# powei-lin/aprilgrid-rs

Hardware: AMD Instinct MI355X
Metric: Mpix/s through the saddle chain (blur->threshold->gradient->saddle), frames resident in HBM (higher is better)
Workload: dtype f32; 1 GPU; configs[1]: 256 synthetic 1280x800 L8 AprilGrid frames per GPU (T36H11 6x6 board, seeded renderer, frame indices 0..255 per rank: 256 distinct); frames_per_gpu=256, width=1280, height=800, format=L8, distinct_frames_per_gpu=256, parallelism=1 GPU, steps_per_gather=1, batches_in_flight=1

## Files before the change

### aprilgrid-rs_amd/csrc/chain_kernels.h

```cpp
#pragma once
#include <cstddef>
#include <cstdint>

namespace agx {

enum Kernel : int {
    K_BLUR_HESSIAN = 0,
    K_THRESHOLD = 1,
    K_FLOOD_REFINE = 2,
    K_RARE = 3,
    K_SPARSE = 4,
    K_COUNT = 5
};

struct RefinedRec {
    uint32_t key;
    float x, y, k, theta, phi;
};

struct FrameCounters {
    uint32_t min_key_inv;
    uint32_t pad0[31];
    uint32_t n_seeds;
    uint32_t n_clusters;
    uint32_t n_refined;
    uint32_t max_k_bits;
    uint32_t flags;
    uint32_t n_out;
    uint32_t out_offset;
    uint32_t n_cand;
    uint32_t n_roots;
    uint32_t n_big;
    uint32_t refine_done;
    uint32_t n_clusters2;
    uint32_t stats[20];
};
static_assert(sizeof(FrameCounters) == 256, "FrameCounters is cleared as 64 dwords");
enum : uint32_t {
    FLAG_CAND_OVERFLOW = 1u,
    FLAG_ROOT_OVERFLOW = 2u,
    FLAG_OUT_OVERFLOW = 4u,
    FLAG_CENTROID_INEXACT = 8u,
    FLAG_BIG_CLUSTER = 16u,
    FLAG_RING_BELOW = 32u,
    FLAG_LARGE_RESULT = 64u
};

struct RefineConsts {
    float cone[25];
    float pmat[150];
};

struct ChainArgs {
    const uint8_t *frames;
    long long frame_stride;
    int row_stride;
    int byte_rows;
    int fmt;
    int W, H, n_frames;
    long long plane;
    int threads;
    int n_strips;
    int strip_cols;
    int rows_per_seg;
    int n_segs;
    int k1_group;
    int k1_async_poll;
    float publish_factor;
    float w[7];
    float *blur;
    float *resp_dbg;
    float *dummy;
    float *cand_max;
    uint32_t *slot_plane;
    uint32_t *mask;
    int mask_wpr;
    int mask_yb;
    long long mask_plane;
    int force_generic;
    int sparse_after_verify;
    unsigned long long *wave_times;
    int dbg;
    FrameCounters *ctr;
    FrameCounters *ctr_next;
    uint32_t *total_out;
    uint32_t cap_cand, cap_roots, cap_out;
    uint32_t *seeds;
    uint32_t *clu_key;
    uint32_t *clu_cnt;
    uint32_t *clu_sx, *clu_sy;
    uint32_t *cand;
    uint32_t *parent;
    unsigned long long *sumx, *sumy;
    uint32_t *cnt, *minidx;
    uint32_t *roots;
    RefinedRec *refined;
    float *out;
    uint32_t out_total_cap;
    uint32_t *frame_table;
    float min_angle, max_angle;
};

int tuning_env(const char *name, int dflt);
void tuning_env_reload();

bool plan_k1(ChainArgs &a, int override_rows_per_seg);

int launch_kernel(int which, const ChainArgs &a, const RefineConsts &rc, void *stream, bool deferred_refine = false);

struct RefinePointsArgs {
    const float *img;
    long long frame_stride;
    long long pitch;
    int W, H;
    int padded;
    const float *points;
    uint32_t points_per_frame;
    const uint32_t *counts;
    float *out;
    uint32_t *status;
};
int launch_refine_points(const RefinePointsArgs &p, const RefineConsts &rc, int n_frames, void *stream);

constexpr int REFINE_PATCH_MAX_HALF = 4;
constexpr int REFINE_PATCH_MAX_TAPS = (2 * REFINE_PATCH_MAX_HALF + 1) * (2 * REFINE_PATCH_MAX_HALF + 1);
struct RefinePatchConsts {
    float cone[REFINE_PATCH_MAX_TAPS];
    float pmat[REFINE_PATCH_MAX_TAPS * 6];
};
int launch_refine_patch(const RefinePointsArgs &p, const RefinePatchConsts *consts, int half, int n_frames, void *stream);

int launch_generic_cluster(const ChainArgs &a, void *stream);
int launch_refine_clusters(const ChainArgs &a, const RefinePatchConsts *consts, int half, void *stream);

size_t k5_lds_bytes(const ChainArgs &a);

constexpr size_t WAVE_TIMES_STRIDE = (size_t)1 << 20;

constexpr int MASK_PAD_X = 64;

int init_device_kernels();

int launch_debug_resp(const ChainArgs &a, int frame, float *dst, void *stream);
int launch_publish(const ChainArgs &a, uint32_t h_out_records, uint32_t *h_table_dev, float *h_out_dev, void *stream);
int launch_clear_counters(FrameCounters *ctr, size_t n_records, void *stream);
int launch_front_luma(const void *src, size_t row_stride, size_t frame_stride, int n_frames, int format, void *dst, int out8, int W,
                      int H, void *stream);
int launch_luma8(const void *src, size_t pitch, size_t frame_stride, int n_frames, int format, uint8_t *dst, int W, int H,
                 void *stream);


constexpr int GB_MAX_RADIUS = 16;
constexpr int GB_TX = 64, GB_TY = 64;
constexpr int GB_HPITCH = GB_TX + 1;
struct GaussBlurArgs {
    const uint8_t *src;
    long long src_frame_stride;
    int src_row_stride;
    int W, H;
    float *dst;
    long long dst_frame_stride;
    long long dst_row_stride;
    int radius;
    float w[2 * GB_MAX_RADIUS + 1];
};
size_t gauss_blur_lds_bytes(int radius);
int launch_gauss_blur(const GaussBlurArgs &a, int format, int n_frames, void *stream);

struct HessianArgs {
    const uint8_t *src;
    long long src_frame_stride;
    int src_row_stride;
    int W, H;
    float *dst;
    long long dst_frame_stride, dst_row_stride;
};
int launch_hessian_response(const HessianArgs &a, int format, int n_frames, void *stream);

int launch_response_front(const ChainArgs &a, void *stream);

struct PlaneFrontArgs {
    const float *src;
    long long frame_stride;
    long long row_stride;
};
int launch_plane_front(const ChainArgs &a, const PlaneFrontArgs &p, void *stream);

constexpr uint32_t EMIT_CLUSTERS_MAX = 16384;
struct EmitClustersArgs {
    uint32_t per_frame;
    uint32_t *rows;
    float *points;
    uint32_t *counts;
    uint32_t *status;
};
int launch_emit_clusters(const ChainArgs &a, const EmitClustersArgs &e, void *stream);

struct FilterSaddlesArgs {
    const float *records;
    uint32_t *status;
    const uint32_t *counts;
    uint32_t per_frame;
    float min_angle, max_angle;
    uint32_t filtered;
};
int launch_filter_saddles(const FilterSaddlesArgs &f, int n_frames, void *stream);

}
```

### aprilgrid-rs_amd/csrc/chain_kernels.hip

```cpp
#include <hip/hip_runtime.h>

#include <map>
#include <mutex>
#include <string>

#include "chain_kernels.h"

namespace agx {

__device__ __forceinline__ uint32_t f32_order_key(float f)
{
    uint32_t u = __float_as_uint(f);
    return (u & 0x80000000u) ? ~u : (u | 0x80000000u);
}
__device__ __forceinline__ float f32_from_order_key(uint32_t key)
{
    uint32_t u = (key & 0x80000000u) ? (key & 0x7fffffffu) : ~key;
    return __uint_as_float(u);
}

template <int D>
__device__ __forceinline__ float div_const(float v)
{
    const float r = 1.0f / (float)D;
// ... 642 lines not shown
                            s_def[wv][y - ys][lane_id_here()] = pk;
                        }
                        if (cj_any != 0ull && !defer_row) {
                            float sel[4];
#pragma unroll
                            for (int j = 0; j < 4; ++j)
                                asm("v_cndmask_b32_e64 %0, %1, %2, %3" : "=v"(sel[j]) : "v"(cmax), "v"(dv[j]), "s"(cj[j]));
                            cmax = fmaxf(fmaxf(cmax, sel[0]), sel[1]);
                            cmax = fmaxf(fmaxf(cmax, sel[2]), sel[3]);
                        }
                    }
                    y_pushed = y;
                }
                if (__builtin_expect((y & 31) == 31 || y == ye - 1, 0)) {
                    const int ln = lane_id_here();
                    const int c0h = xs - 4 + 4 * ln;
                    auto store_block = [&](int yb, const uint32_t (&w)[4], float m) {
                        if (c0h >= xs && c0h < xe) {
                            a.cand_max[((size_t)frame * a.mask_yb + yb) * (a.mask_wpr >> 2) + ((MASK_PAD_X + c0h) >> 2)] = m;
                            uint32_t *dst = mask_f + (size_t)yb * a.mask_wpr + MASK_PAD_X + c0h;
                            if (A4) {
                                *reinterpret_cast<uint4 *>(dst) = make_uint4(w[0], w[1], w[2], w[3]);
                            } else {
#pragma unroll
                                for (int j = 0; j < 4; ++j)
                                    if (c0h + j < W) dst[j] = w[j];
                            }
                        }
                    };
                    auto refilter = [&](uint32_t (&w)[4], float &m) {
                        const float thr_now = __builtin_bit_cast(float, thr_run_bits);
                        const int q_lo = ys < 1 ? 1 - ys : 0;
                        const int q_hi = min(K1_DEFER_ROWS, min(ye, H - 1) - ys);
#pragma unroll 1
                        for (int q = q_lo; q < q_hi; ++q) {
                            const uint2 pk = s_def[wv][q][ln];
#pragma unroll
                            for (int j = 0; j < 4; ++j) {
                                const uint32_t half = j < 2 ? pk.x : pk.y;
                                const uint32_t raw = (j & 1) ? (half & 0xffff0000u) : (half << 16);
                                const float hi = __uint_as_float(raw), lo = __uint_as_float(raw | 0xffffu);
                                const bool bit = ((w[j] >> q) & 1u) != 0u;
                                const bool keep = bit && lo < thr_now;
                                if (bit && !keep) w[j] &= ~(1u << q);
                                if (keep) m = fmaxf(m, hi);
                            }
                        }
                    };
                    const int blk = (y >> 5) - (ys >> 5);
                    if (DEFER && blk == 1) {
                        uint32_t o0[4];
#pragma unroll
                        for (int j = 0; j < 4; ++j) o0[j] = s_blk0[wv][j][ln];
                        float cm0 = __uint_as_float(s_blk0[wv][4][ln]);
                        refilter(o0, cm0);
                        store_block((y >> 5) - 1, o0, cm0);
                    }
                    const int fix = 31 - (y_pushed & 31);
#pragma unroll
                    for (int j = 0; j < 4; ++j) mw[j] = __brev(mw[j]) >> fix;
                    if (DEFER && blk == 0 && y != ye - 1) {
#pragma unroll
                        for (int j = 0; j < 4; ++j) s_blk0[wv][j][ln] = mw[j];
                        s_blk0[wv][4][ln] = __float_as_uint(cmax);
                    } else {
                        if (DEFER && blk == 0) refilter(mw, cmax);
                        store_block(y >> 5, mw, cmax);
                    }
                    mw[0] = mw[1] = mw[2] = mw[3] = 0u;
                    cmax = -__builtin_inff();
                }
            }
            up = mid;
            mid = dn;
        }
    }
    const float run_min = wave_min_f32(lane_min());
    if (async_poll) polled = __builtin_amdgcn_readfirstlane(polled_v);
    else if (first_sync) asm volatile("s_waitcnt lgkmcnt(0)" : "+s"(polled) : : "memory");
    const bool known_smaller = polled != 0u && !(run_min < f32_from_order_key(~polled));
    if (lane == 0 && !known_smaller) atomicMax(&ctr.min_key_inv, ~f32_order_key(run_min));
}

__device__ __forceinline__ float det_at(const float *c, int W)
{
    const float v11 = c[-W - 1], v12 = c[-W], v13 = c[-W + 1];
    const float v21 = c[-1], v22 = c[0], v23 = c[1];
    const float v31 = c[W - 1], v32 = c[W], v33 = c[W + 1];
    const float t22 = v22 * 2.0f;
    const float lxx = (v21 - t22) + v23;
    const float lyy = (v12 - t22) + v32;
    const float lxy = (((v13 - v11) + v31) - v33) * 0.25f;
    return lxx * lyy - lxy * lxy;
}

__device__ __forceinline__ uint32_t retest_word(const float *blur, int W, int yb, int x, uint32_t m0, float thr)
{
    uint32_t m = m0, keep = m0;
    const float *col = blur + (size_t)(yb * 32) * W + x;
    while (m) {
        int b[4];
        b[0] = __ffs(m) - 1;
        m &= m - 1;
#pragma unroll
        for (int q = 1; q < 4; ++q) {
            b[q] = m ? __ffs(m) - 1 : b[q - 1];
            m &= m - 1;
        }
        float d[4];
#pragma unroll
        for (int q = 0; q < 4; ++q) d[q] = det_at(col + (size_t)b[q] * W, W);
#pragma unroll
        for (int q = 0; q < 4; ++q)
            if (!(d[q] < thr)) keep &= ~(1u << b[q]);
    }
    return keep;
}

constexpr int VS_OWN = 56;
constexpr int VS_ROWS = 4;
constexpr uint32_t VS_LIST = 512;

#ifndef AGX_VS_ATTR
#define AGX_VS_ATTR __attribute__((amdgpu_num_sgpr(80), amdgpu_waves_per_eu(8, 8)))
#endif
#ifndef AGX_VS_WAVES
#define AGX_VS_WAVES 1
#endif
constexpr int VS_WAVES = AGX_VS_WAVES;
#ifndef AGX_VS_RT
#define AGX_VS_RT 2
#endif
constexpr int VS_RT = AGX_VS_RT;
__device__ __forceinline__ void wave_lds_sync()
{
    __builtin_amdgcn_fence(__ATOMIC_RELEASE, "wavefront");
    __builtin_amdgcn_wave_barrier();
    __builtin_amdgcn_fence(__ATOMIC_ACQUIRE, "wavefront");
}

constexpr uint32_t SEED_LDS_CAP = 4096;
struct FrameLds {
    uint32_t *n_seeds, *flags;
    uint32_t *seeds;
};

__device__ __forceinline__ uint32_t seed_bits(uint32_t kw, uint32_t upw)
{
    uint32_t sd = kw & ~from_left_u(kw) & ~upw;
    uint32_t alive = sd, mk = kw, uk = upw;
#pragma unroll
    for (int k = 1; k < 8; ++k) {
        if (!__any(alive != 0u)) break;
        mk = from_right_u(mk);
        uk = from_right_u(uk);
        alive &= mk;
        const uint32_t kill = alive & uk;
        sd &= ~kill;
        alive &= ~kill;
    }
    return sd;
}

constexpr uint32_t K2_DBG_BITS = 32u | 64u | 128u | 256u | 2048u | 8192u;
template <bool DBG, bool GRID3 = false>
__device__ __forceinline__ void verify_tiles(const ChainArgs &a, int frame, int first_tile, int tile_stride, uint32_t *s_keep,
                                             uint32_t *s_list)
{
    const uint32_t dbg = DBG ? a.dbg : 0u;
    FrameCounters &ctr = a.ctr[frame];
    uint32_t *mask = a.mask + (size_t)frame * (size_t)a.mask_plane;
    const float *blur = a.blur + (size_t)frame * (size_t)a.plane;
    const float *cmax_f = a.cand_max + (size_t)frame * (size_t)a.mask_yb * (size_t)(a.mask_wpr >> 2);
    const int W = a.W, wpr = a.mask_wpr;
    const int lane = threadIdx.x & 63;
    const int n_yb = (a.H + 31) >> 5;
    const int groups = GRID3 ? (int)gridDim.y : (W + VS_OWN - 1) / VS_OWN;
    const int tiles = GRID3 ? first_tile + 1 : ((n_yb + VS_ROWS - 1) / VS_ROWS) * groups;
    const bool phase_on = (dbg & 8192) != 0;
    unsigned long long t_prev = phase_on ? wall_clock64() : 0ull;
    auto phase = [&](int which) {
        if (phase_on) {
            const unsigned long long now = wall_clock64();
            if (lane == 0) atomicAdd(&ctr.stats[which], (uint32_t)(now - t_prev));
            t_prev = now;
        }
    };
    for (int t = first_tile; t < tiles; t += tile_stride) {
        const int ch = GRID3 ? (int)blockIdx.z : t / groups, g = GRID3 ? (int)blockIdx.y : t - ch * groups;
        const int yb0 = ch * VS_ROWS;
        const int x = g * VS_OWN - 1 + lane;
        uint32_t *wp0 = mask + (size_t)yb0 * wpr + MASK_PAD_X + x;
        const size_t cm_col = (size_t)((MASK_PAD_X + x) >> 2);
        uint32_t m[VS_ROWS];
#pragma unroll
        for (int r = 0; r < VS_ROWS; ++r) m[r] = wp0[(size_t)r * wpr];
        const int up_row = yb0 > 0 ? -1 : 0;
        uint32_t uword = wp0[(ptrdiff_t)up_row * wpr];
        float cm_pre[VS_ROWS];
#pragma unroll
        for (int r = 0; r < VS_ROWS; ++r) cm_pre[r] = cmax_f[(size_t)(yb0 + r) * (wpr >> 2) + cm_col];
        float cmu_pre = cmax_f[(size_t)(yb0 + up_row) * (wpr >> 2) + cm_col];
        uint32_t min_key_inv = ctr.min_key_inv;
        asm volatile("" : "+v"(m[0]), "+v"(m[1]), "+v"(m[2]), "+v"(m[3]), "+v"(uword), "+v"(cm_pre[0]), "+v"(cm_pre[1]), "+v"(cm_pre[2]),
                     "+v"(cm_pre[3]), "+v"(cmu_pre), "+v"(min_key_inv));
        const float thr = f32_from_order_key(~min_key_inv) * 0.05f;
        static_assert(VS_ROWS == 4, "the asm above names the tile's four rows");
        if (yb0 == 0) uword = 0u;
        uint32_t any = 0u;
#pragma unroll
        for (int r = 0; r < VS_ROWS; ++r) any |= m[r];
        const bool tile_empty = !__any(any != 0u);
        phase(0);
        if (phase_on && lane == 0) atomicAdd(&ctr.stats[tile_empty ? 6 : 7], 1u);
        if (tile_empty) continue;
        float cm[VS_ROWS];
#pragma unroll
        for (int r = 0; r < VS_ROWS; ++r) cm[r] = m[r] ? cm_pre[r] : -__builtin_inff();
        const bool up_need = (m[0] & 1u) && (uword >> 31);
        const float cmu = up_need ? cmu_pre : -__builtin_inff();
        uint32_t needmask = 0u;
#pragma unroll
        for (int r = 0; r < VS_ROWS; ++r)
            if (m[r] && !(cm[r] < thr)) needmask |= 1u << r;
        const bool up_retest = up_need && !(cmu < thr);
        if (phase_on) { (void)__any(needmask != 0u || up_retest); phase(1); }
        if (dbg & 128) {
            const bool own = lane >= 1 && lane <= VS_OWN && x < W;
#pragma unroll
            for (int r = 0; r < VS_ROWS; ++r)
                if (own && m[r]) {
                    const int q = (yb0 + r) & 3;
                    atomicAdd(&ctr.stats[q * 4 + 0], 1u);
                    atomicAdd(&ctr.stats[q * 4 + 1], (uint32_t)__popc(m[r]));
                    if (needmask & (1u << r)) {
                        atomicAdd(&ctr.stats[q * 4 + 2], 1u);
                        atomicAdd(&ctr.stats[q * 4 + 3], (uint32_t)__popc(m[r]));
                    }
                }
        }
        if (dbg & 2048) {
            const bool own = lane >= 1 && lane <= VS_OWN && x < W;
#pragma unroll
            for (int r = 0; r < VS_ROWS; ++r)
                if (own && (needmask & (1u << r))) {
                    const int q = (yb0 + r) & 3, sg = (yb0 + r) >> 2;
                    atomicAdd(&ctr.stats[16 + (sg < 3 ? sg : 3)], (uint32_t)__popc(m[r]));
                    if (q == 0)
                        for (int h = 0; h < 16; ++h) atomicAdd(&ctr.stats[h], (uint32_t)__popc(m[r] & (3u << (2 * h))));
                }
        }
        uint32_t keep[VS_ROWS];
#pragma unroll
        for (int r = 0; r < VS_ROWS; ++r) keep[r] = m[r];
        uint32_t upbit = up_need ? 1u : 0u;
        const unsigned long long need_any = __ballot(needmask != 0u || up_retest);
        if (need_any && !(dbg & 32)) {
            const uint32_t rows_any = wave_or_u32(needmask);
            uint32_t n_list = 0;
            auto run_list = [&]() {
                wave_lds_sync();
                for (uint32_t e0 = 0; e0 < n_list; e0 += 64 * VS_RT) {
                    float d[VS_RT];
                    uint32_t ent[VS_RT];
                    bool on[VS_RT];
#pragma unroll
                    for (int q = 0; q < VS_RT; ++q) {
                        const uint32_t e = e0 + q * 64 + (uint32_t)lane;
                        on[q] = e < n_list;
                        ent[q] = s_list[on[q] ? e : 0u];
                        const int ln = (int)((ent[q] >> 5) & 63u), r = (int)(ent[q] >> 11), b = (int)(ent[q] & 31u);
                        const int row = r == VS_ROWS ? yb0 * 32 - 1 : (yb0 + r) * 32 + b;
                        d[q] = (dbg & 256) ? 0.0f : det_at(blur + (size_t)row * W + (g * VS_OWN - 1 + ln), W);
                    }
#pragma unroll
                    for (int q = 0; q < VS_RT; ++q)
                        if (on[q] && !(d[q] < thr)) atomicAnd(&s_keep[ent[q] >> 5], ~(1u << (ent[q] & 31u)));
                }
                wave_lds_sync();
                n_list = 0;
            };
            auto push = [&](bool mine, uint32_t entry) {
                const unsigned long long bal = __ballot(mine);
                const uint32_t k = (uint32_t)__popcll(bal);
                if (n_list + k > VS_LIST) run_list();
                if (mine) s_list[n_list + __builtin_amdgcn_mbcnt_hi((uint32_t)(bal >> 32), __builtin_amdgcn_mbcnt_lo((uint32_t)bal, 0u))] = entry;
                n_list += k;
            };
            s_keep[VS_ROWS * 64 + lane] = 1u;
            if (__any(up_retest)) push(up_retest, (uint32_t)(VS_ROWS * 64 + lane) << 5);
#pragma unroll
            for (int r = 0; r < VS_ROWS; ++r) {
                if (!(rows_any & (1u << r))) continue;
                s_keep[r * 64 + lane] = m[r];
                const uint32_t mr = (needmask & (1u << r)) ? m[r] : 0u;
                uint32_t bits_any = wave_or_u32(mr);
                while (bits_any) {
                    const int b = __builtin_ctz(bits_any);
                    bits_any &= bits_any - 1;
                    push((mr >> b) & 1u, ((uint32_t)(r * 64 + lane) << 5) | (uint32_t)b);
                }
            }
            if (n_list) run_list();
#pragma unroll
            for (int r = 0; r < VS_ROWS; ++r)
                if (rows_any & (1u << r)) keep[r] = s_keep[r * 64 + lane];
            if (up_retest) upbit = s_keep[VS_ROWS * 64 + lane] & 1u;
        }
        phase(2);
        const bool owner = lane >= 1 && lane <= VS_OWN && x < W;
#pragma unroll
        for (int r = 0; r < VS_ROWS; ++r)
            if (owner && keep[r] != m[r]) wp0[(size_t)r * wpr] = keep[r];
        if (dbg & 128) {
#pragma unroll
            for (int r = 0; r < VS_ROWS; ++r)
                if (owner && m[r]) atomicAdd(&ctr.stats[16 + ((yb0 + r) & 3)], (uint32_t)__popc(keep[r]));
        }
        uint32_t carry = upbit;
        if (dbg & 64) continue;
        uint32_t sdr[VS_ROWS], c = 0u;
#pragma unroll
        for (int r = 0; r < VS_ROWS; ++r) {
            const uint32_t kw = keep[r];
            const uint32_t upw = (kw << 1) | carry;
            carry = kw >> 31;
            sdr[r] = 0u;
            if (__any(kw != 0u)) {
                const uint32_t sd = seed_bits(kw, upw);
                sdr[r] = owner ? sd : 0u;
            }
            c += (uint32_t)__popc(sdr[r]);
        }
        phase(3);
        if (__any(c != 0u)) {
            static_assert(VS_ROWS == 4, "two packed scans");
            const uint32_t c01 = (uint32_t)__popc(sdr[0]) | ((uint32_t)__popc(sdr[1]) << 16), c23 = (uint32_t)__popc(sdr[2]) | ((uint32_t)__popc(sdr[3]) << 16);
            const uint32_t i01 = wave_incl_scan_u32(c01), i23 = wave_incl_scan_u32(c23);
            const uint32_t t01 = (uint32_t)__builtin_amdgcn_readlane((int)i01, 63), t23 = (uint32_t)__builtin_amdgcn_readlane((int)i23, 63);
            const uint32_t tot[VS_ROWS] = {t01 & 0xffffu, t01 >> 16, t23 & 0xffffu, t23 >> 16};
            const uint32_t exc[VS_ROWS] = {(i01 - c01) & 0xffffu, (i01 - c01) >> 16, (i23 - c23) & 0xffffu, (i23 - c23) >> 16};
            uint32_t base = 0u;
            if (lane == 0) base = atomicAdd(&ctr.n_seeds, tot[0] + tot[1] + tot[2] + tot[3]);
            base = (uint32_t)__builtin_amdgcn_readfirstlane((int)base);
            if (phase_on) phase(4);
#pragma unroll
            for (int r = 0; r < VS_ROWS; ++r) {
                uint32_t sd = sdr[r], o = base + exc[r];
                base += tot[r];
                while (sd) {
                    const int b = __ffs(sd) - 1;
                    sd &= sd - 1;
                    const uint32_t pix = (uint32_t)((yb0 + r) * 32 + b) * (uint32_t)W + (uint32_t)x;
                    if (o < a.cap_roots) a.seeds[(size_t)frame * a.cap_roots + o] = pix;
                    else atomicOr(&ctr.flags, FLAG_CAND_OVERFLOW);
                    ++o;
                }
            }
        }
        phase(5);
    }
}

template <bool DBG, bool GRID3 = false>
__global__ void __launch_bounds__(64 * VS_WAVES) AGX_VS_ATTR k_verify_seeds(ChainArgs a)
{
    static_assert(!GRID3 || VS_WAVES == 1, "one tile per workgroup");
    __shared__ uint32_t s_keep_all[VS_WAVES][(VS_ROWS + 1) * 64];
    __shared__ uint32_t s_list_all[VS_WAVES][VS_LIST];
    const int wv = __builtin_amdgcn_readfirstlane((int)(threadIdx.x >> 6));
    const WaveTimer wt(a, K_THRESHOLD, DBG);
    if (GRID3) {
        verify_tiles<DBG, true>(a, a.n_frames - 1 - (int)blockIdx.x, 0, 1, s_keep_all[0], s_list_all[0]);
        return;
    }
    FrameSlot fs = frame_slot(a.n_frames, true);
    fs.slot = fs.slot * VS_WAVES + (uint32_t)wv;
    fs.n_slots *= VS_WAVES;
    verify_tiles<DBG>(a, fs.frame, (int)fs.slot, (int)fs.n_slots, s_keep_all[wv], s_list_all[wv]);
}

constexpr int VF_TB = 4;
constexpr uint32_t VFW_SLOTS = 256;
constexpr uint32_t VFW_LIST = 512;
constexpr uint32_t VFW_WORDS = 3 * VFW_SLOTS + VFW_LIST;
struct VerifyLds {
    uint32_t *idx, *pix, *keep;
    uint32_t *list;
};

__device__ __forceinline__ void verify_frame(const ChainArgs &a, int frame, const VerifyLds &vl)
{
    const uint32_t t = threadIdx.x;
    const int lane = (int)(t & 63u);
    const int wv = __builtin_amdgcn_readfirstlane((int)(t >> 6));
    FrameCounters &ctr = a.ctr[frame];
    uint32_t *mask = a.mask + (size_t)frame * (size_t)a.mask_plane;
    const float *blur = a.blur + (size_t)frame * (size_t)a.plane;
    const float *cmax_f = a.cand_max + (size_t)frame * (size_t)a.mask_yb * (size_t)(a.mask_wpr >> 2);
    const int W = a.W, wpr = a.mask_wpr;
    const int n_yb = (a.H + 31) >> 5;
    const int n_ch = (n_yb + VS_ROWS - 1) / VS_ROWS;
    const float thr = f32_from_order_key(~ctr.min_key_inv) * 0.05f;
    auto stamp = [&](int which) {
        if ((a.dbg & 131072) && t == 0) ctr.stats[which] = (uint32_t)wall_clock64();
    };
    const bool wclk = (a.dbg & 131072) && wv == 0;
    unsigned long long t_prev = wclk ? wall_clock64() : 0ull;
    auto wphase = [&](int which) {
        if (wclk) {
            const unsigned long long now = wall_clock64();
            if (lane == 0) ctr.stats[8 + which] += (uint32_t)(now - t_prev);
            t_prev = now;
        }
    };
    uint32_t n_list = 0, n_slots = 0;
    auto run_list = [&]() {
        wphase(1);
        wave_lds_sync();
        constexpr int EB = 4;
        for (uint32_t e0 = 0; e0 < n_list; e0 += 64u * EB) {
            float d[EB];
            uint32_t ent[EB];
            bool on[EB];
#pragma unroll
            for (int k = 0; k < EB; ++k) {
                const uint32_t e = e0 + (uint32_t)k * 64u + (uint32_t)lane;
                on[k] = e < n_list;
                ent[k] = vl.list[on[k] ? e : 0u];
                d[k] = (a.dbg & 256) ? 0.0f : det_at(blur + (size_t)vl.pix[ent[k] >> 5] + (size_t)(ent[k] & 31u) * W, W);
            }
#pragma unroll
            for (int k = 0; k < EB; ++k)
                if (on[k] && !(d[k] < thr)) atomicAnd(&vl.keep[ent[k] >> 5], ~(1u << (ent[k] & 31u)));
        }
        wave_lds_sync();
        n_list = 0;
        wphase(2);
    };
    auto flush_slots = [&]() {
        run_list();
        for (uint32_t sl = (uint32_t)lane; sl < n_slots; sl += 64u) mask[vl.idx[sl]] = vl.keep[sl];
        wave_lds_sync();
        n_slots = 0;
        wphase(3);
    };
    auto push = [&](bool mine, uint32_t entry) {
        const unsigned long long bal = __ballot(mine);
        const uint32_t k = (uint32_t)__popcll(bal);
        if (n_list + k > VFW_LIST) run_list();
        if ((a.dbg & 131072) && lane == 0) atomicAdd(&ctr.stats[14], k);
        if (mine) vl.list[n_list + __builtin_amdgcn_mbcnt_hi((uint32_t)(bal >> 32), __builtin_amdgcn_mbcnt_lo((uint32_t)bal, 0u))] = entry;
        n_list += k;
    };
    {
        const int groups = (W + 63) >> 6;
        const int tiles = n_ch * groups;
        for (int tb = wv; tb < tiles && !(a.dbg & 32); tb += 16 * VF_TB) {
            uint32_t m[VF_TB][VS_ROWS];
            float cm[VF_TB][VS_ROWS];
#pragma unroll
            for (int k = 0; k < VF_TB; ++k) {
// ... 396 lines not shown
        const uint32_t lm = wp[-1];
        const uint32_t um = (m << 1) | (yb > 0 ? (wp[-wpr] >> 31) : 0u);
        while (m) {
            const int b = __ffs(m) - 1;
            m &= m - 1;
            const uint32_t p = (uint32_t)(yb * 32 + b) * (uint32_t)W + (uint32_t)x;
            const uint32_t slot = atomicAdd(&ctr.n_cand, 1u);
            if (slot < a.cap_cand) {
                const size_t o = base + slot;
                a.cand[o] = p | (((lm >> b) & 1u) << 30) | (((um >> b) & 1u) << 31);
                a.parent[o] = slot;
                a.sumx[o] = 0ull;
                a.sumy[o] = 0ull;
                a.cnt[o] = 0u;
                a.minidx[o] = 0xffffffffu;
                slot_plane[p] = slot;
            } else {
                atomicOr(&ctr.flags, FLAG_CAND_OVERFLOW);
            }
        }
    }
    phase_barrier();
    const uint32_t n = __hip_atomic_load(&ctr.n_cand, __ATOMIC_RELAXED, __HIP_MEMORY_SCOPE_AGENT);
    if (n > a.cap_cand) {
        if (t == 0) ctr.n_clusters = ctr.n_clusters2 = 0u;
        return;
    }
    for (uint32_t s = t; s < n; s += T) {
        const uint32_t e = a.cand[base + s];
        const uint32_t p = e & 0x3fffffffu;
        if (e & 0x40000000u) uf_unite(parent, s, slot_plane[p - 1]);
        if (e & 0x80000000u) uf_unite(parent, s, slot_plane[p - a.W]);
    }
    phase_barrier();
    for (uint32_t s = t; s < n; s += T) {
        const uint32_t p = a.cand[base + s] & 0x3fffffffu;
        const uint32_t r = uf_find_atomic(parent, s);
        atomicAdd(&a.sumx[base + r], (unsigned long long)(p % (uint32_t)a.W));
        atomicAdd(&a.sumy[base + r], (unsigned long long)(p / (uint32_t)a.W));
        atomicAdd(&a.cnt[base + r], 1u);
        atomicMin(&a.minidx[base + r], p);
        if (r == s) {
            uint32_t i = atomicAdd(&ctr.n_roots, 1u);
            if (i < a.cap_roots) a.roots[(size_t)frame * a.cap_roots + i] = s;
            else atomicOr(&ctr.flags, FLAG_ROOT_OVERFLOW);
        }
    }
    phase_barrier();
    const uint32_t nr = min(__hip_atomic_load(&ctr.n_roots, __ATOMIC_RELAXED, __HIP_MEMORY_SCOPE_AGENT), a.cap_roots);
    for (uint32_t i = t; i < nr; i += T) {
        const uint32_t s = __hip_atomic_load(&a.roots[(size_t)frame * a.cap_roots + i], __ATOMIC_RELAXED, __HIP_MEMORY_SCOPE_AGENT);
        const size_t q = (size_t)frame * a.cap_roots + i;
        a.clu_key[q] = __hip_atomic_load(&a.minidx[base + s], __ATOMIC_RELAXED, __HIP_MEMORY_SCOPE_AGENT);
        a.clu_cnt[q] = __hip_atomic_load(&a.cnt[base + s], __ATOMIC_RELAXED, __HIP_MEMORY_SCOPE_AGENT);
        a.clu_sx[q] = (uint32_t)__hip_atomic_load(&a.sumx[base + s], __ATOMIC_RELAXED, __HIP_MEMORY_SCOPE_AGENT);
        a.clu_sy[q] = (uint32_t)__hip_atomic_load(&a.sumy[base + s], __ATOMIC_RELAXED, __HIP_MEMORY_SCOPE_AGENT);
    }
    if (t == 0) {
        ctr.n_clusters = nr;
        ctr.n_clusters2 = 0u;
    }
}


__device__ __forceinline__ void generic_sums(const ChainArgs &a, int frame, uint32_t i, unsigned long long &sx, unsigned long long &sy)
{
    const size_t base = (size_t)frame * a.cap_cand;
    const uint32_t s = __hip_atomic_load(&a.roots[(size_t)frame * a.cap_roots + i], __ATOMIC_RELAXED, __HIP_MEMORY_SCOPE_AGENT);
    sx = __hip_atomic_load(&a.sumx[base + s], __ATOMIC_RELAXED, __HIP_MEMORY_SCOPE_AGENT);
    sy = __hip_atomic_load(&a.sumy[base + s], __ATOMIC_RELAXED, __HIP_MEMORY_SCOPE_AGENT);
}


__device__ __forceinline__ float hessian_det(float v11, float v12, float v13, float v21, float v22, float v23, float v31, float v32,
                                             float v33)
{
    const float t22 = v22 * 2.0f;
    const float lxx = (v21 - t22) + v23;
    const float lyy = (v12 - t22) + v32;
    const float lxy = (((v13 - v11) + v31) - v33) * 0.25f;
    return lxx * lyy - lxy * lxy;
}

__global__ void k_debug_resp(const float *__restrict__ blur, float *__restrict__ resp, int W, int H)
{
    const long long n = (long long)W * H;
    for (long long i = (long long)blockIdx.x * blockDim.x + threadIdx.x; i < n; i += (long long)gridDim.x * blockDim.x) {
        const int x = (int)(i % W), y = (int)(i / W);
        float d = 0.0f;
        if (x > 0 && x < W - 1 && y > 0 && y < H - 1) {
            const float *c = blur + i;
            d = hessian_det(c[-W - 1], c[-W], c[-W + 1], c[-1], c[0], c[1], c[W - 1], c[W], c[W + 1]);
        }
        resp[i] = d;
    }
}

constexpr uint32_t TAIL_CAP = 1024;
struct RecSinkGlobal {
    uint32_t *n_refined, *max_k_bits, *flags;
    __device__ __forceinline__ void put(const ChainArgs &a, int frame, uint32_t o, const uint32_t (&f)[6]) const
    {
        uint32_t *rec = reinterpret_cast<uint32_t *>(a.refined + (size_t)frame * a.cap_roots + o);
#pragma unroll
        for (int q = 0; q < 6; ++q) __hip_atomic_store(rec + q, f[q], __ATOMIC_RELAXED, __HIP_MEMORY_SCOPE_AGENT);
    }
};
struct RecSinkLds {
    uint32_t *n_refined, *max_k_bits, *flags;
    uint32_t *rec;
    __device__ __forceinline__ void put(const ChainArgs &a, int frame, uint32_t o, const uint32_t (&f)[6]) const
    {
        if (o < TAIL_CAP) {
#pragma unroll
            for (int q = 0; q < 6; ++q) rec[q * TAIL_CAP + o] = f[q];
        }
        uint32_t *g = reinterpret_cast<uint32_t *>(a.refined + (size_t)frame * a.cap_roots + o);
#pragma unroll
        for (int q = 0; q < 6; ++q) g[q] = f[q];
    }
};

template <bool VEC, typename CLK, typename SINK, typename SUM>
__device__ __forceinline__ void refine_values(const ChainArgs &a, const RefineConsts &rc, int frame, const float *img, int W, int H,
                                              uint32_t key, uint32_t cn, SUM sx, SUM sy, const SINK &sink, float &cx,
                                              float &cy, CLK &clk)
{
    if (sx >= (1u << 24) || sy >= (1u << 24)) atomicOr(sink.flags, FLAG_CENTROID_INEXACT);
    const float fn = (float)cn;
    const float initial_x = (float)sx / fn;
    const float initial_y = (float)sy / fn;
    cx = initial_x;
    cy = initial_y;
    const float rxf = roundf(initial_x), ryf = roundf(initial_y);
    const int round_x = (int)rxf, round_y = (int)ryf;
    if (round_y - 4 < 0 || round_y + 4 >= H || round_x - 4 < 0 || round_x + 4 >= W) return;
    const int wx0 = round_x - 4;
    const int al = VEC ? (wx0 & 3) : 0;
    const float *win = img + (size_t)(round_y - 4) * W + (wx0 - al);
    float conv[25];
#pragma unroll
    for (int q = 0; q < 25; ++q) conv[q] = 0.0f;
    float prm[6] = {0.0f, 0.0f, 0.0f, 0.0f, 0.0f, 0.0f};
    constexpr int NQ = VEC ? 3 : 9;
    typedef float rowload_t __attribute__((ext_vector_type(VEC ? 4 : 1)));
    rowload_t raw[5][NQ];
    auto fetch = [&](int first, int n) {
#pragma unroll
        for (int k = 0; k < 5; ++k)
            if (k < n) {
#pragma unroll
                for (int e = 0; e < NQ; ++e)
                    raw[k][e] = *reinterpret_cast<const rowload_t *>(win + (size_t)(first + k) * W + (VEC ? 4 * e : e));
            }
        asm volatile("" ::: "memory");
    };
    fetch(0, 5);
    if (CLK::on) {
        asm volatile("s_waitcnt vmcnt(0)" ::: "memory");
        clk.mark(11);
    }
#pragma unroll
    for (int wr = 0; wr < 9; ++wr) {
        if (wr == 5) {
            clk.mark(12);
            fetch(5, 4);
            if (CLK::on) {
                asm volatile("s_waitcnt vmcnt(0)" ::: "memory");
                clk.mark(13);
            }
        }
        float v[9];
        const int k = wr < 5 ? wr : wr - 5;
        if (VEC) {
            const rowload_t q0 = raw[k][0], q1 = raw[k][1 % NQ], q2 = raw[k][2 % NQ];
            const bool s1 = (al & 1) != 0, s2 = (al & 2) != 0;
            const float u0 = s1 ? q0[1 % (VEC ? 4 : 1)] : q0[0], u1 = s1 ? q0[2 % (VEC ? 4 : 1)] : q0[1 % (VEC ? 4 : 1)], u2 = s1 ? q0[3 % (VEC ? 4 : 1)] : q0[2 % (VEC ? 4 : 1)], u3 = s1 ? q1[0] : q0[3 % (VEC ? 4 : 1)];
            const float u4 = s1 ? q1[1 % (VEC ? 4 : 1)] : q1[0], u5 = s1 ? q1[2 % (VEC ? 4 : 1)] : q1[1 % (VEC ? 4 : 1)], u6 = s1 ? q1[3 % (VEC ? 4 : 1)] : q1[2 % (VEC ? 4 : 1)], u7 = s1 ? q2[0] : q1[3 % (VEC ? 4 : 1)];
            const float u8 = s1 ? q2[1 % (VEC ? 4 : 1)] : q2[0], u9 = s1 ? q2[2 % (VEC ? 4 : 1)] : q2[1 % (VEC ? 4 : 1)], u10 = s1 ? q2[3 % (VEC ? 4 : 1)] : q2[2 % (VEC ? 4 : 1)];
            v[0] = s2 ? u2 : u0; v[1] = s2 ? u3 : u1; v[2] = s2 ? u4 : u2; v[3] = s2 ? u5 : u3; v[4] = s2 ? u6 : u4;
            v[5] = s2 ? u7 : u5; v[6] = s2 ? u8 : u6; v[7] = s2 ? u9 : u7; v[8] = s2 ? u10 : u8;
        } else {
#pragma unroll
            for (int e = 0; e < 9; ++e) v[e] = raw[k][e % NQ][0];
        }
#pragma unroll
        for (int r = 0; r < 5; ++r) {
            const int pr = wr - r;
            if (pr < 0 || pr > 4) continue;
#pragma unroll
            for (int c = 0; c < 5; ++c)
#pragma unroll
                for (int pc = 0; pc < 5; ++pc) conv[r * 5 + c] = conv[r * 5 + c] + v[c + pc] * rc.cone[pr * 5 + pc];
        }
        if (wr >= 4) {
            const int r = wr - 4;
#pragma unroll
            for (int c = 0; c < 5; ++c)
#pragma unroll
                for (int j = 0; j < 6; ++j) prm[j] = prm[j] + rc.pmat[(r * 5 + c) * 6 + j] * conv[r * 5 + c];
        }
    }
    if (CLK::on) {
        asm volatile("" : "+v"(prm[0]), "+v"(prm[1]), "+v"(prm[2]), "+v"(prm[3]), "+v"(prm[4]), "+v"(prm[5]));
        clk.mark(16);
    }
    const float a1 = prm[0], a2 = prm[1], a3 = prm[2], a4 = prm[3], a5 = prm[4];
    const float fxx = 2.0f * a1, fyy = 2.0f * a3, fxy = a2;
    const float d = fxx * fyy - fxy * fxy;
    if (!(d < 0.0f)) return;
    float x0, y0;
    {
        const float A0 = 2.0f * a1, B0 = a2, R0 = -a4;
        const float A1 = a2, B1 = 2.0f * a3, R1 = -a5;
        float pa, pb, pr_, qa, qb, qr;
        if (fabsf(A1) > fabsf(A0)) {
            pa = A1; pb = B1; pr_ = R1; qa = A0; qb = B0; qr = R0;
        } else {
            pa = A0; pb = B0; pr_ = R0; qa = A1; qb = B1; qr = R1;
        }
        const float l = qa / pa;
        const float u22 = qb - l * pb;
        const float y2 = qr - l * pr_;
        y0 = y2 / u22;
        x0 = (pr_ - pb * y0) / pa;
    }
    if (!(fabsf(x0) <= 1.0f && fabsf(y0) <= 1.0f)) return;
    const float c5 = (a1 + a3) / 2.0f;
    const float c4 = (a1 - a3) / 2.0f;
    const float c3 = a2 / 2.0f;
    const float k = sqrtf(c4 * c4 + c3 * c3);
    if (!(fabsf(c5) < k)) return;
    const float PI_F = 3.14159274101257324219f;
    const float phi = acosf(-c5 / k) / 2.0f / PI_F * 180.0f;
    const float theta = atan2f(c3, c4) / 2.0f / PI_F * 180.0f;
    if (CLK::on) {
        float th = theta, ph = phi;
        asm volatile("" : "+v"(th), "+v"(ph));
        clk.mark(17);
    }
    uint32_t o = atomicAdd(sink.n_refined, 1u);
    if (CLK::on) {
        asm volatile("" : "+v"(o));
        clk.mark(15);
    }
    if (o >= a.cap_roots) return;
    const uint32_t f[6] = {key, __float_as_uint(rxf + x0), __float_as_uint(ryf + y0),
                           __float_as_uint(k),  __float_as_uint(theta),     __float_as_uint(phi)};
    sink.put(a, frame, o, f);
    atomicMax(sink.max_k_bits, __float_as_uint(k));
}

template <typename SUM>
__device__ __forceinline__ void cluster_centroid(uint32_t *flags, uint32_t cn, SUM sx, SUM sy, float &cx, float &cy)
{
    if (sx >= (1u << 24) || sy >= (1u << 24)) atomicOr(flags, FLAG_CENTROID_INEXACT);
    const float fn = (float)cn;
    cx = (float)sx / fn;
    cy = (float)sy / fn;
}

template <bool VEC>
__device__ __forceinline__ void refine_cluster(const ChainArgs &a, const RefineConsts &rc, int frame, size_t cbase,
                                               const float *img, int W, int H, uint32_t s, uint32_t *n_refined,
                                               uint32_t *max_k_bits)
{
    float cx, cy;
    NoClock clk;
    const RecSinkGlobal sink{n_refined, max_k_bits, &a.ctr[frame].flags};
    unsigned long long sx, sy;
    generic_sums(a, frame, s, sx, sy);
    refine_values<VEC>(a, rc, frame, img, W, H, a.clu_key[cbase + s], a.clu_cnt[cbase + s], sx, sy, sink, cx, cy, clk);
    a.clu_sx[cbase + s] = __float_as_uint(cx);
    a.clu_sy[cbase + s] = __float_as_uint(cy);
}

template <bool VEC, typename CLK, bool REFINE = true>
__global__ void __launch_bounds__(64) __attribute__((amdgpu_waves_per_eu(AGX_FLOOD_WPE, 8))) k_flood_refine(ChainArgs a, RefineConsts rc)
{
    const WaveTimer wt(a, K_FLOOD_REFINE);
    const FrameSlot fs = frame_slot(a.n_frames, true);
    const int frame = fs.frame;
    FrameCounters &ctr = a.ctr[frame];
    if (a.force_generic) return;
    const size_t cbase = (size_t)frame * a.cap_roots;
    const int lane = threadIdx.x;
    CLK clk;
    clk.start(ctr.stats);
    uint32_t flags0 = ctr.flags, n_seeds0 = ctr.n_seeds;
    const uint32_t i0 = fs.slot * 64u + (uint32_t)lane;
    uint32_t p0 = i0 < a.cap_roots ? a.seeds[cbase + i0] : 0u;
    asm volatile("" : "+v"(flags0), "+v"(n_seeds0), "+v"(p0));
    if (flags0 & FLAG_CAND_OVERFLOW) return;
    const uint32_t n = min(n_seeds0, a.cap_roots);
    const uint32_t *mask = a.mask + (size_t)frame * (size_t)a.mask_plane;
    const float *img = a.blur + (size_t)frame * (size_t)a.plane;
    const uint32_t W = (uint32_t)a.W;
    for (uint32_t base = fs.slot * 64u; base < n; base += fs.n_slots * 64u) {
        const uint32_t i = base + (uint32_t)lane;
        uint32_t p = 0u, cnt = 0, sumx = 0, sumy = 0;
        int what = FLOOD_NONE;
        if (CLK::on && lane == 0) atomicAdd(&ctr.stats[19], 1u);
        clk.mark(8);
        if (i < n) {
            p = base == fs.slot * 64u ? p0 : a.seeds[cbase + i];
            what = flood_lane(a, mask, W, p, cnt, sumx, sumy, clk);
        }
        clk.join();
        clk.mark(10);
        unsigned long long big = __ballot(what == FLOOD_BIG);
        if (big && lane == 0) atomicAdd(&ctr.n_big, (uint32_t)__popcll(big));
        while (big) {
            const int src = __ffsll((long long)big) - 1;
            big &= big - 1ull;
            uint32_t c2 = 0, x2 = 0, y2 = 0;
            const int w2 = wave_flood_128x64(a, &ctr.flags, mask, (uint32_t)__builtin_amdgcn_readlane((int)p, src), lane, c2, x2, y2);
            if (lane == src) {
                what = w2 == FLOOD_CLUSTER ? FLOOD_CLUSTER : FLOOD_NONE;
                cnt = c2;
                sumx = x2;
                sumy = y2;
            }
        }
        clk.mark(14);
        if (CLK::on) {
            const unsigned long long act = __ballot(what == FLOOD_CLUSTER);
            if (lane == 0) atomicAdd(&ctr.stats[18], (uint32_t)__popcll(act));
        }
        if (what == FLOOD_CLUSTER) {
            const uint32_t o = atomicAdd(&ctr.n_clusters, 1u);
            float cx, cy;
            if constexpr (REFINE) {
                const RecSinkGlobal sink{&ctr.n_refined, &ctr.max_k_bits, &ctr.flags};
                refine_values<VEC>(a, rc, frame, img, a.W, a.H, p, cnt, sumx, sumy, sink, cx, cy, clk);
            } else {
                cluster_centroid(&ctr.flags, cnt, sumx, sumy, cx, cy);
            }
            if (o < a.cap_roots) {
                a.clu_key[cbase + o] = p;
                a.clu_cnt[cbase + o] = cnt;
                a.clu_sx[cbase + o] = __float_as_uint(cx);
                a.clu_sy[cbase + o] = __float_as_uint(cy);
            } else {
                atomicOr(&ctr.flags, FLAG_ROOT_OVERFLOW);
            }
        }
        clk.join();
        clk.mark(7);
    }
}

__device__ __forceinline__ void filter_sort_emit(const ChainArgs &a, int frame, uint32_t n, uint32_t max_k_bits,
                                                 uint32_t *keys, uint32_t *idxs, uint32_t lds_entries, uint32_t *s_count,
                                                 uint32_t *s_offset, uint32_t *s_fits)
{
// ... 121 lines not shown
            uint32_t *row = a.frame_table + (size_t)frame * 4;
            const uint32_t flags = __hip_atomic_load(&ctr.flags, __ATOMIC_RELAXED, __HIP_MEMORY_SCOPE_AGENT);
            const bool bad = (flags & (FLAG_CAND_OVERFLOW | FLAG_ROOT_OVERFLOW | FLAG_OUT_OVERFLOW)) != 0;
            row[0] = bad ? 0u : nf;
            row[1] = off;
            row[2] = flags;
            row[3] = __hip_atomic_load(&ctr.n_clusters, __ATOMIC_RELAXED, __HIP_MEMORY_SCOPE_AGENT) +
                     __hip_atomic_load(&ctr.n_clusters2, __ATOMIC_RELAXED, __HIP_MEMORY_SCOPE_AGENT);
        }
    }
    __syncthreads();
    if (!pass || !s_misc[1]) return;
    float *out = a.out + (size_t)s_misc[0] * 5;
#pragma unroll
    for (int q = 0; q < 5; ++q) out[(size_t)rank * 5 + q] = __uint_as_float(f[q + 1]);
}

__device__ __forceinline__ void emit_wide_lds(const ChainArgs &a, int frame, uint32_t n, uint32_t max_k_bits, const uint32_t *rec,
                                              uint32_t *keys, uint32_t *s_misc, uint32_t *flags_lds, uint32_t n_clusters)
{
    const uint32_t t = threadIdx.x;
    FrameCounters &ctr = a.ctr[frame];
    const float s_max_k = __uint_as_float(max_k_bits) / 10.0f;
    uint32_t f[6] = {0xffffffffu, 0u, 0u, 0u, 0u, 0u};
    bool pass = false;
    if (t < n) {
#pragma unroll
        for (int q = 0; q < 6; ++q) f[q] = rec[q * TAIL_CAP + t];
        const float k = __uint_as_float(f[3]), phi = __uint_as_float(f[5]);
        pass = k >= s_max_k && phi >= a.min_angle && phi <= a.max_angle;
    }
    keys[t] = pass ? f[0] : 0xffffffffu;
    if (t < 4) keys[TAIL_CAP + t] = 0xffffffffu;
    const uint32_t nf = (uint32_t)__syncthreads_count(pass ? 1 : 0);
    const bool ok = nf <= a.cap_out;
    uint32_t off = 0;
    if (t == 0 && ok && nf) off = atomicAdd(a.total_out, nf);
    const uint32_t n4 = (n + 3u) >> 2;
    uint32_t rank = 0;
    if (pass) {
        for (uint32_t j = 0; j < n4; ++j) {
            const uint4 q = reinterpret_cast<const uint4 *>(keys)[j];
            rank += (q.x < f[0] ? 1u : 0u) + (q.y < f[0] ? 1u : 0u) + (q.z < f[0] ? 1u : 0u) + (q.w < f[0] ? 1u : 0u);
        }
    }
    if (t == 0) {
        uint32_t fits = 1;
        if (ok && nf && off + nf > a.out_total_cap) fits = 0;
        if (!ok || !fits) *flags_lds |= FLAG_OUT_OVERFLOW;
        s_misc[0] = off;
        s_misc[1] = (ok && fits) ? 1u : 0u;
        ctr.n_out = nf;
        ctr.out_offset = off;
        if (a.frame_table) {
            uint32_t *row = a.frame_table + (size_t)frame * 4;
            const uint32_t flags = *flags_lds;
            const bool bad = (flags & (FLAG_CAND_OVERFLOW | FLAG_ROOT_OVERFLOW | FLAG_OUT_OVERFLOW)) != 0;
            row[0] = bad ? 0u : nf;
            row[1] = off;
            row[2] = flags;
            row[3] = n_clusters;
        }
    }
    __syncthreads();
    if (!pass || !s_misc[1]) return;
    float *out = a.out + (size_t)s_misc[0] * 5;
#pragma unroll
    for (int q = 0; q < 5; ++q) out[(size_t)rank * 5 + q] = __uint_as_float(f[q + 1]);
}

struct FrameHead {
    uint32_t flags, n_refined, max_k_bits;
};
__device__ __forceinline__ FrameHead load_frame_head(const FrameCounters &ctr)
{
    FrameHead h;
    h.flags = __hip_atomic_load(&ctr.flags, __ATOMIC_RELAXED, __HIP_MEMORY_SCOPE_AGENT);
    h.n_refined = __hip_atomic_load(&ctr.n_refined, __ATOMIC_RELAXED, __HIP_MEMORY_SCOPE_AGENT);
    h.max_k_bits = __hip_atomic_load(&ctr.max_k_bits, __ATOMIC_RELAXED, __HIP_MEMORY_SCOPE_AGENT);
    asm volatile("" : "+v"(h.flags), "+v"(h.n_refined), "+v"(h.max_k_bits));
    return h;
}

template <bool EMIT_ONLY = false>
__device__ __forceinline__ void rare_frame(const ChainArgs &a, const RefineConsts &rc, int frame, uint32_t *lds_u, uint32_t lds_entries,
                                           uint32_t *s_misc3, const FrameHead &head)
{
    uint32_t &s_count = s_misc3[0], &s_offset = s_misc3[1], &s_fits = s_misc3[2];
    FrameCounters &ctr = a.ctr[frame];
    uint32_t flags0 = head.flags, n_ref0 = head.n_refined, maxk0 = head.max_k_bits;
    const bool generic = !EMIT_ONLY && (a.force_generic || (flags0 & FLAG_BIG_CLUSTER));
    const size_t cbase = (size_t)frame * a.cap_roots;
    const float *img = a.blur + (size_t)frame * (size_t)a.plane;
    if (generic) {
        generic_frame(a, frame);
        if (threadIdx.x == 0) {
            __hip_atomic_store(&ctr.n_refined, 0u, __ATOMIC_RELAXED, __HIP_MEMORY_SCOPE_AGENT);
            __hip_atomic_store(&ctr.max_k_bits, 0u, __ATOMIC_RELAXED, __HIP_MEMORY_SCOPE_AGENT);
        }
        phase_barrier();
        const uint32_t flags = __hip_atomic_load(&ctr.flags, __ATOMIC_RELAXED, __HIP_MEMORY_SCOPE_AGENT);
        if (!(flags & (FLAG_CAND_OVERFLOW | FLAG_ROOT_OVERFLOW))) {
            const uint32_t n = min(__hip_atomic_load(&ctr.n_clusters, __ATOMIC_RELAXED, __HIP_MEMORY_SCOPE_AGENT), a.cap_roots);
            for (uint32_t i = threadIdx.x; i < n; i += blockDim.x)
                refine_cluster<false>(a, rc, frame, cbase, img, a.W, a.H, i, &ctr.n_refined, &ctr.max_k_bits);
        }
        phase_barrier();
    }
    if (generic) {
        flags0 = __hip_atomic_load(&ctr.flags, __ATOMIC_RELAXED, __HIP_MEMORY_SCOPE_AGENT);
        n_ref0 = __hip_atomic_load(&ctr.n_refined, __ATOMIC_RELAXED, __HIP_MEMORY_SCOPE_AGENT);
        maxk0 = __hip_atomic_load(&ctr.max_k_bits, __ATOMIC_RELAXED, __HIP_MEMORY_SCOPE_AGENT);
    }
    const bool void_frame = (flags0 & (FLAG_CAND_OVERFLOW | FLAG_ROOT_OVERFLOW)) != 0;
    const uint32_t n_ref = void_frame ? 0u : n_ref0;
    const uint32_t maxk = maxk0;
    if (n_ref <= TAIL_CAP && lds_entries * 2 >= TAIL_CAP + 8) {
        emit_wide(a, frame, n_ref, maxk, lds_u, &s_count);
        return;
    }
    if (threadIdx.x == 0) atomicOr(&ctr.flags, FLAG_LARGE_RESULT);
    __syncthreads();
    if (n_ref <= lds_entries) {
        filter_sort_emit(a, frame, n_ref, maxk, lds_u, lds_u + lds_entries, lds_entries, &s_count, &s_offset, &s_fits);
    } else {
        filter_sort_emit(a, frame, n_ref, maxk, a.seeds + (size_t)frame * a.cap_roots, a.roots + (size_t)frame * a.cap_roots,
                         a.cap_roots, &s_count, &s_offset, &s_fits);
    }
}

__device__ __forceinline__ void clear_next_counters(const ChainArgs &a, int frame)
{
    if (a.ctr_next && threadIdx.x < 64) {
        reinterpret_cast<uint32_t *>(&a.ctr_next[frame])[threadIdx.x] = 0u;
        if (frame == 0) reinterpret_cast<uint32_t *>(&a.ctr_next[a.n_frames])[threadIdx.x] = 0u;
    }
}

__device__ __forceinline__ bool emit_large_split(const ChainArgs &a, int frame, uint32_t part, uint32_t n_parts, uint32_t n, uint32_t max_k_bits,
                                                 uint32_t *keys, uint32_t *idxs, uint32_t lds_entries, uint32_t *s_cnt )
{
    const uint32_t t = threadIdx.x, T = blockDim.x;
    FrameCounters &ctr = a.ctr[frame];
    uint32_t *rec = reinterpret_cast<uint32_t *>(a.refined + (size_t)frame * a.cap_roots);
    auto rec_u = [&](uint32_t i, int field) { return __hip_atomic_load(rec + (size_t)i * 6 + field, __ATOMIC_RELAXED, __HIP_MEMORY_SCOPE_AGENT); };
    if (t < n_parts + 2) s_cnt[t] = 0u;
    __syncthreads();
    const float s_max_k = __uint_as_float(max_k_bits) / 10.0f;
    const unsigned long long plane = (unsigned long long)a.plane;
    for (uint32_t i = t; i < n; i += T) {
        const float k = __uint_as_float(rec_u(i, 3)), phi = __uint_as_float(rec_u(i, 5));
        if (k >= s_max_k && phi >= a.min_angle && phi <= a.max_angle) {
            const uint32_t key = rec_u(i, 0);
            const uint32_t band = (uint32_t)(((unsigned long long)key * n_parts) / plane);
            const uint32_t o = atomicAdd(&s_cnt[band], 1u);
            if (band == part && o < lds_entries) {
                keys[o] = key;
                idxs[o] = i;
            }
        }
    }
    __syncthreads();
    uint32_t nf = 0, below = 0, biggest = 0;
    for (uint32_t b = 0; b < n_parts; ++b) {
        const uint32_t c = s_cnt[b];
        if (b < part) below += c;
        nf += c;
        biggest = max(biggest, c);
    }
    uint32_t need = 1;
    while (need < biggest) need <<= 1;
    if (need > lds_entries) return false;
    const uint32_t mine = s_cnt[part];
    if (t == 0) {
        uint32_t off = 0, fits = 1;
        const uint32_t won = atomicCAS(&ctr.refine_done, 0u, 1u);
        if (won == 0u) {
            const bool ok = nf <= a.cap_out;
            if (ok && nf) {
                off = atomicAdd(a.total_out, nf);
                if (off + nf > a.out_total_cap) fits = 0;
            }
            if (!ok || !fits) atomicOr(&ctr.flags, FLAG_OUT_OVERFLOW);
            ctr.n_out = nf;
            ctr.out_offset = off;
            if (a.frame_table) {
                uint32_t *row = a.frame_table + (size_t)frame * 4;
                const uint32_t flags = __hip_atomic_load(&ctr.flags, __ATOMIC_RELAXED, __HIP_MEMORY_SCOPE_AGENT) | FLAG_LARGE_RESULT;
// ... 17 lines not shown
    __syncthreads();
    if (!s_cnt[n_parts + 1] || !mine) return true;
    uint32_t np2 = 1;
    while (np2 < mine) np2 <<= 1;
    for (uint32_t i = mine + t; i < np2; i += T) {
        keys[i] = 0xffffffffu;
        idxs[i] = 0;
    }
    __syncthreads();
    for (uint32_t k2 = 2; k2 <= np2; k2 <<= 1) {
        for (uint32_t j = k2 >> 1; j > 0; j >>= 1) {
            for (uint32_t i = t; i < np2; i += T) {
                const uint32_t l = i ^ j;
                if (l > i) {
                    const bool asc = (i & k2) == 0;
                    const uint32_t ki = keys[i], kl = keys[l];
                    if ((ki > kl) == asc) {
                        keys[i] = kl; keys[l] = ki;
                        const uint32_t ti = idxs[i]; idxs[i] = idxs[l]; idxs[l] = ti;
                    }
                }
            }
            __syncthreads();
        }
    }
    float *out = a.out + ((size_t)s_cnt[n_parts] + below) * 5;
    for (uint32_t i = t; i < mine; i += T) {
        const uint32_t src = idxs[i];
#pragma unroll
        for (int q = 0; q < 5; ++q) out[(size_t)i * 5 + q] = __uint_as_float(rec_u(src, q + 1));
    }
    return true;
}

constexpr uint32_t RARE_MAX_PARTS = 8;
template <bool EMIT_ONLY>
__device__ __forceinline__ void rare_parts(const ChainArgs &a, const RefineConsts &rc, uint32_t lds_entries, uint32_t n_parts,
                                           uint32_t *lds_u, uint32_t *s_misc3, uint32_t *s_cnt )
{
    const WaveTimer wt(a, K_RARE);
    const int frame = (int)(blockIdx.x / n_parts);
    const uint32_t part = blockIdx.x - (uint32_t)frame * n_parts;
    if (part == 0) clear_next_counters(a, frame);
    FrameCounters &ctr = a.ctr[frame];
    const FrameHead head = load_frame_head(ctr);
    if (n_parts > 1) {
        const bool generic = !EMIT_ONLY && (a.force_generic || (head.flags & FLAG_BIG_CLUSTER));
        const bool void_frame = (head.flags & (FLAG_CAND_OVERFLOW | FLAG_ROOT_OVERFLOW)) != 0;
        const bool split = !generic && !void_frame && head.n_refined > TAIL_CAP;
        if (split) {
            if (part == 0 && threadIdx.x == 0) atomicOr(&ctr.flags, FLAG_LARGE_RESULT);
            if (emit_large_split(a, frame, part, n_parts, head.n_refined, head.max_k_bits, lds_u, lds_u + lds_entries, lds_entries, s_cnt)) return;
            __syncthreads();
        }
        if (part != 0) return;
    }
    rare_frame<EMIT_ONLY>(a, rc, frame, lds_u, lds_entries, s_misc3, head);
}
__global__ void __launch_bounds__(1024) k_rare(ChainArgs a, RefineConsts rc, uint32_t lds_entries, uint32_t n_parts)
{
    extern __shared__ __attribute__((aligned(16))) uint32_t lds_u[];
    __shared__ uint32_t s_misc3[3];
    __shared__ uint32_t s_cnt[RARE_MAX_PARTS + 2];
    rare_parts<false>(a, rc, lds_entries, n_parts, lds_u, s_misc3, s_cnt);
}
__global__ void __launch_bounds__(1024) k_rare_emit_only(ChainArgs a, RefineConsts rc, uint32_t lds_entries, uint32_t n_parts)
{
    extern __shared__ __attribute__((aligned(16))) uint32_t lds_u[];
    __shared__ uint32_t s_misc3[3];
    __shared__ uint32_t s_cnt[RARE_MAX_PARTS + 2];
    rare_parts<true>(a, rc, lds_entries, n_parts, lds_u, s_misc3, s_cnt);
}

constexpr uint32_t SF_MISC = 16;
constexpr uint32_t SF_REC = SF_MISC;
constexpr uint32_t SF_R = SF_REC + 6 * TAIL_CAP;
constexpr uint32_t SF_R_WORDS = 16 * VFW_WORDS;
constexpr uint32_t SF_WORDS = SF_R + SF_R_WORDS;
static_assert(SF_R_WORDS >= TAIL_CAP + 8 && SF_R_WORDS >= SEED_LDS_CAP, "the emission's keys and the flood path's seeds fit the shared region");
static_assert(SF_REC % 4 == 0 && SF_R % 4 == 0, "16-byte aligned parts");
static_assert(SF_WORDS * 4 <= 160 * 1024 - 1024, "fits a CU's LDS");
enum : int { SFM_SEEDS = 0, SFM_FLAGS = 1, SFM_CLUSTERS = 2, SFM_REFINED = 3, SFM_MAXK = 4, SFM_BIG = 5, SFM_EMIT = 8, SFM_RARE = 12 };

template <bool VEC, typename CLK>
__global__ void __launch_bounds__(1024) k_sparse_frame(ChainArgs a, RefineConsts rc, uint32_t lds_entries)
{
    extern __shared__ __attribute__((aligned(16))) uint32_t lds_u[];
    const int frame = a.n_frames - 1 - (int)blockIdx.x;
    const uint32_t t = threadIdx.x;
    const int lane = (int)(t & 63u);
    const int wv = __builtin_amdgcn_readfirstlane((int)(t >> 6));
    clear_next_counters(a, frame);
    uint32_t *misc = lds_u;
    if (t < SF_MISC) misc[t] = 0u;
    __syncthreads();
    FrameCounters &ctr = a.ctr[frame];
    auto stamp = [&](int which) {
        if ((a.dbg & 131072) && t == 0) ctr.stats[which] = (uint32_t)wall_clock64();
    };
    stamp(0);
    const FrameLds fl{&misc[SFM_SEEDS], &misc[SFM_FLAGS], lds_u + SF_R};
    const size_t cbase = (size_t)frame * a.cap_roots;
    const float *img = a.blur + (size_t)frame * (size_t)a.plane;
    const RecSinkLds sink{&misc[SFM_REFINED], &misc[SFM_MAXK], &misc[SFM_FLAGS], lds_u + SF_REC};
    if (a.sparse_after_verify) {
        if (t == 0) {
            misc[SFM_SEEDS] = __hip_atomic_load(&ctr.n_seeds, __ATOMIC_RELAXED, __HIP_MEMORY_SCOPE_AGENT);
            misc[SFM_FLAGS] = __hip_atomic_load(&ctr.flags, __ATOMIC_RELAXED, __HIP_MEMORY_SCOPE_AGENT);
        }
        __syncthreads();
    } else {
        uint32_t *wl = lds_u + SF_R + (uint32_t)wv * VFW_WORDS;
        verify_frame(a, frame, VerifyLds{wl, wl + VFW_SLOTS, wl + 2 * VFW_SLOTS, wl + 3 * VFW_SLOTS});
    }
    stamp(1);
    if (!a.sparse_after_verify) {
        frame_seeds(a, frame, fl);
        __syncthreads();
    }
    stamp(5);
    const uint32_t n_seeds_raw = misc[SFM_SEEDS];
    if (!a.force_generic && n_seeds_raw <= a.cap_roots && !(misc[SFM_FLAGS] & FLAG_CAND_OVERFLOW)) {
        const uint32_t n = n_seeds_raw;
        const uint32_t *mask = a.mask + (size_t)frame * (size_t)a.mask_plane;
        const uint32_t W = (uint32_t)a.W;
        CLK clk;
        clk.start(ctr.stats);
        for (uint32_t base = (uint32_t)wv * 64u; base < n; base += 1024u) {
            const uint32_t i = base + (uint32_t)lane;
            uint32_t p = 0u, cnt = 0, sumx = 0, sumy = 0;
            int what = FLOOD_NONE;
            if (CLK::on && lane == 0) atomicAdd(&ctr.stats[19], 1u);
            clk.mark(8);
            if (i < n) {
                p = (i < SEED_LDS_CAP && !a.sparse_after_verify) ? fl.seeds[i] : a.seeds[cbase + i];
                what = flood_lane(a, mask, W, p, cnt, sumx, sumy, clk);
            }
            clk.join();
            clk.mark(10);
            unsigned long long big = __ballot(what == FLOOD_BIG);
            if (big && lane == 0) atomicAdd(&misc[SFM_BIG], (uint32_t)__popcll(big));
            while (big) {
                const int src = __ffsll((long long)big) - 1;
                big &= big - 1ull;
                uint32_t c2 = 0, x2 = 0, y2 = 0;
                const int w2 = wave_flood_128x64(a, &misc[SFM_FLAGS], mask, (uint32_t)__builtin_amdgcn_readlane((int)p, src), lane, c2, x2, y2);
                if (lane == src) {
                    what = w2 == FLOOD_CLUSTER ? FLOOD_CLUSTER : FLOOD_NONE;
                    cnt = c2;
                    sumx = x2;
                    sumy = y2;
                }
            }
            clk.mark(14);
            if (CLK::on) {
                const unsigned long long act = __ballot(what == FLOOD_CLUSTER);
                if (lane == 0) atomicAdd(&ctr.stats[18], (uint32_t)__popcll(act));
            }
            if (what == FLOOD_CLUSTER) {
                const uint32_t o = atomicAdd(&misc[SFM_CLUSTERS], 1u);
                float cx, cy;
                refine_values<VEC>(a, rc, frame, img, a.W, a.H, p, cnt, sumx, sumy, sink, cx, cy, clk);
                if (o < a.cap_roots) {
                    a.clu_key[cbase + o] = p;
                    a.clu_cnt[cbase + o] = cnt;
                    a.clu_sx[cbase + o] = __float_as_uint(cx);
                    a.clu_sy[cbase + o] = __float_as_uint(cy);
                } else {
                    atomicOr(&misc[SFM_FLAGS], FLAG_ROOT_OVERFLOW);
                }
            }
            clk.join();
            clk.mark(7);
        }
    }
    __syncthreads();
    stamp(2);
    const uint32_t flags = misc[SFM_FLAGS], n_ref = misc[SFM_REFINED], n_clu = min(misc[SFM_CLUSTERS], a.cap_roots);
    const bool void_frame = (flags & (FLAG_CAND_OVERFLOW | FLAG_ROOT_OVERFLOW)) != 0;
    const bool generic = a.force_generic || (flags & FLAG_BIG_CLUSTER);
    if (t == 0) {
        ctr.n_seeds = min(n_seeds_raw, a.cap_roots);
        ctr.n_big = misc[SFM_BIG];
        ctr.n_clusters = n_clu;
        ctr.n_refined = n_ref;
        ctr.max_k_bits = misc[SFM_MAXK];
    }
    if (generic || (!void_frame && n_ref > TAIL_CAP)) {
        if (t == 0) atomicOr(&ctr.flags, flags);
        phase_barrier();
        rare_frame(a, rc, frame, lds_u + SF_MISC, lds_entries, &misc[SFM_RARE], load_frame_head(ctr));
        return;
    }
    emit_wide_lds(a, frame, void_frame ? 0u : n_ref, misc[SFM_MAXK], lds_u + SF_REC, lds_u + SF_R, &misc[SFM_EMIT], &misc[SFM_FLAGS], n_clu);
    if (t == 0) ctr.flags = misc[SFM_FLAGS];
    stamp(3);
}

namespace {
std::mutex g_env_mutex;
std::map<std::string, std::pair<bool, int>, std::less<>> g_env_cache;
}
int tuning_env(const char *name, int dflt)
{
    std::lock_guard<std::mutex> lk(g_env_mutex);
    auto it = g_env_cache.find(name);
    if (it == g_env_cache.end()) {
        const char *s = getenv(name);
        it = g_env_cache.emplace(name, std::make_pair(s && *s, (s && *s) ? atoi(s) : 0)).first;
    }
    return it->second.first ? it->second.second : dflt;
}
void tuning_env_reload()
{
    std::lock_guard<std::mutex> lk(g_env_mutex);
    g_env_cache.clear();
}
static int env_int(const char *name, int dflt) { return tuning_env(name, dflt); }

constexpr long long K1_ASYNC_POLL_MAX_WAVES = 4608;
bool plan_k1(ChainArgs &a, int override_rows_per_seg)
{
    const int W = a.W, H = a.H;
    if (W < 2 || H < 2) return false;
    int n_strips = (W + 247) / 248;
    int strip_cols = (((W + n_strips - 1) / n_strips) + 3) & ~3;
    const int aligned_cols = (strip_cols + 31) & ~31;
    if (aligned_cols <= 248 && (W + aligned_cols - 1) / aligned_cols == n_strips) strip_cols = aligned_cols;
    const int forced_cols = env_int("AGX_K1_STRIP_COLS", 0);
    if (forced_cols >= 4 && forced_cols <= 248 && (forced_cols & 3) == 0) strip_cols = forced_cols;
    n_strips = (W + strip_cols - 1) / strip_cols;
    a.n_strips = n_strips;
    a.strip_cols = strip_cols;
    a.threads = 256;
    int rps = override_rows_per_seg > 0 ? override_rows_per_seg : env_int("AGX_K1_ROWS", 0);
    if (rps <= 0) {
        const long long target_waves = 10240;
        long long segs = (target_waves + (long long)a.n_frames * n_strips - 1) / ((long long)a.n_frames * n_strips);
        if (segs < 1) segs = 1;
        rps = (int)((H + segs - 1) / segs);
        if (rps > 96) rps = 96;
    }
    rps = ((rps + 31) / 32) * 32;
    if (rps < 32) rps = 32;
    if (rps > 128) rps = 128;
    a.rows_per_seg = rps;
    a.n_segs = (H + rps - 1) / rps;
    a.publish_factor = a.n_strips * a.n_segs > 128 ? 1.5f : 1.0f;
    a.k1_group = env_int("AGX_K1_GROUP", 0);
    const int ap = env_int("AGX_K1_ASYNC_POLL", -1);
    a.k1_async_poll = ap >= 0 ? (ap != 0) : ((long long)a.n_strips * a.n_segs * a.n_frames <= K1_ASYNC_POLL_MAX_WAVES);
    return true;
}

size_t sparse_frame_lds_bytes(const ChainArgs &a)
{
    return std::max<size_t>((size_t)SF_WORDS * 4, (size_t)SF_MISC * 4 + k5_lds_bytes(a));
}

size_t k5_lds_bytes(const ChainArgs &a)
{
    uint32_t e = 1024;
    while (e < a.cap_out && e < 16384u) e <<= 1;
    return (size_t)e * 8;
}

template <int FMT>
static hipError_t launch_k1(const ChainArgs &a, hipStream_t st)
{
    const long long units = (long long)a.n_strips * a.n_segs * a.n_frames;
    dim3 grid((unsigned)((units + 3) / 4)), block(256);
    const size_t k1_lds = (size_t)env_int("AGX_K1_LDS_KB", 0) * 1024;
    const bool small = a.plane * 4 < (1ll << 31) && (long long)a.H * a.row_stride < (1ll << 31);
    const bool a4 = (a.W & 3) == 0 && small && !a.byte_rows;
    const bool uf = !a4 && small && a.W >= 4 && env_int("AGX_K1_UNALIGNED_FAST", 1) != 0;
    if (uf) {
        if (a.resp_dbg) hipLaunchKernelGGL((k_blur_hessian<FMT, false, true, true>), grid, block, k1_lds, st, a);
        else hipLaunchKernelGGL((k_blur_hessian<FMT, false, false, true>), grid, block, k1_lds, st, a);
        return hipGetLastError();
    }
    if (a.resp_dbg) {
        if (a4) hipLaunchKernelGGL((k_blur_hessian<FMT, true, true>), grid, block, k1_lds, st, a);
        else hipLaunchKernelGGL((k_blur_hessian<FMT, false, true>), grid, block, k1_lds, st, a);
    } else if (a4) hipLaunchKernelGGL((k_blur_hessian<FMT, true>), grid, block, k1_lds, st, a);
    else hipLaunchKernelGGL((k_blur_hessian<FMT, false>), grid, block, k1_lds, st, a);
    return hipGetLastError();
}

static int sparse_grid_x(const ChainArgs &a, int per_frame_default, const char *env = nullptr)
{
    if (env) {
        const int v = env_int(env, 0);
        if (v > 0) return v;
    }
    long long gx = 4096 / (a.n_frames > 0 ? a.n_frames : 1);
    if (gx < per_frame_default) gx = per_frame_default;
    if (gx > 256) gx = 256;
    return (int)gx;
}

int launch_kernel(int which, const ChainArgs &a, const RefineConsts &rc, void *stream, bool deferred_refine)
{
    hipStream_t st = (hipStream_t)stream;
    switch (which) {
    case K_BLUR_HESSIAN:
        if (a.fmt == 0) return launch_k1<0>(a, st);
        if (a.fmt == 1) return launch_k1<1>(a, st);
        if (a.fmt == 3) return launch_k1<3>(a, st);
        return launch_k1<2>(a, st);
    case K_THRESHOLD: {
        const int n_yb = (a.H + 31) >> 5;
        int tiles = ((n_yb + VS_ROWS - 1) / VS_ROWS) * ((a.W + VS_OWN - 1) / VS_OWN);
        if (tiles > 512) tiles = 512;
        const int per_frame = (env_int("AGX_G_VERIFY", tiles) + VS_WAVES - 1) / VS_WAVES;
        dim3 grid((unsigned)per_frame * (unsigned)a.n_frames), block(64 * VS_WAVES);
        if ((a.dbg & K2_DBG_BITS) || a.wave_times) hipLaunchKernelGGL(k_verify_seeds<true>, grid, block, 0, st, a);
        else if (VS_WAVES == 1 && env_int("AGX_G_VERIFY", 0) <= 0 && (n_yb + VS_ROWS - 1) / VS_ROWS <= 65535 && (a.W + VS_OWN - 1) / VS_OWN <= 65535)
            hipLaunchKernelGGL((k_verify_seeds<false, VS_WAVES == 1>), dim3((unsigned)a.n_frames, (unsigned)((a.W + VS_OWN - 1) / VS_OWN), (unsigned)((n_yb + VS_ROWS - 1) / VS_ROWS)),
                               block, 0, st, a);
        else hipLaunchKernelGGL(k_verify_seeds<false>, grid, block, 0, st, a);
        return hipGetLastError();
    }
    case K_FLOOD_REFINE: {
        dim3 grid((unsigned)sparse_grid_x(a, 16, "AGX_G_FLOOD") * (unsigned)a.n_frames), block(64);
        if (deferred_refine) {
            hipLaunchKernelGGL((k_flood_refine<false, NoClock, false>), grid, block, 0, st, a, rc);
        } else if (a.dbg & 16384) {
            if ((a.W & 3) == 0) hipLaunchKernelGGL((k_flood_refine<true, PhaseClock>), grid, block, 0, st, a, rc);
            else hipLaunchKernelGGL((k_flood_refine<false, PhaseClock>), grid, block, 0, st, a, rc);
        } else if ((a.W & 3) == 0) {
            hipLaunchKernelGGL((k_flood_refine<true, NoClock>), grid, block, 0, st, a, rc);
        } else {
            hipLaunchKernelGGL((k_flood_refine<false, NoClock>), grid, block, 0, st, a, rc);
        }
        return hipGetLastError();
    }
    case K_RARE: {
        size_t lds = k5_lds_bytes(a);
        uint32_t parts = a.n_frames >= 128 ? 1u : (a.n_frames >= 64 ? 4u : RARE_MAX_PARTS);
        const int forced = env_int("AGX_RARE_PARTS", 0);
        if (forced >= 1 && forced <= (int)RARE_MAX_PARTS) parts = (uint32_t)forced;
        dim3 grid((unsigned)a.n_frames * parts), block(1024);
        if (deferred_refine) hipLaunchKernelGGL(k_rare_emit_only, grid, block, lds, st, a, rc, (uint32_t)(lds / 8), parts);
        else hipLaunchKernelGGL(k_rare, grid, block, lds, st, a, rc, (uint32_t)(lds / 8), parts);
        return hipGetLastError();
    }
    case K_SPARSE: {
        const size_t lds = sparse_frame_lds_bytes(a);
        dim3 grid(a.n_frames), block(1024);
        const uint32_t le = (uint32_t)(k5_lds_bytes(a) / 8);
        if (a.dbg & 262144) {
            if ((a.W & 3) == 0) hipLaunchKernelGGL((k_sparse_frame<true, PhaseClock>), grid, block, lds, st, a, rc, le);
            else hipLaunchKernelGGL((k_sparse_frame<false, PhaseClock>), grid, block, lds, st, a, rc, le);
        } else if ((a.W & 3) == 0) hipLaunchKernelGGL((k_sparse_frame<true, NoClock>), grid, block, lds, st, a, rc, le);
        else hipLaunchKernelGGL((k_sparse_frame<false, NoClock>), grid, block, lds, st, a, rc, le);
        return hipGetLastError();
    }
    default:
        return hipErrorInvalidValue;
    }
}

int init_device_kernels()
{
    hipError_t e = hipFuncSetAttribute((const void *)k_rare, hipFuncAttributeMaxDynamicSharedMemorySize, 160 * 1024 - 1024);
    if (e == hipSuccess) e = hipFuncSetAttribute((const void *)k_rare_emit_only, hipFuncAttributeMaxDynamicSharedMemorySize, 160 * 1024 - 1024);
    if (e == hipSuccess) e = hipFuncSetAttribute((const void *)k_sparse_frame<true, NoClock>, hipFuncAttributeMaxDynamicSharedMemorySize, 160 * 1024 - 1024);
    if (e == hipSuccess) e = hipFuncSetAttribute((const void *)k_sparse_frame<false, NoClock>, hipFuncAttributeMaxDynamicSharedMemorySize, 160 * 1024 - 1024);
    if (e == hipSuccess) e = hipFuncSetAttribute((const void *)k_sparse_frame<true, PhaseClock>, hipFuncAttributeMaxDynamicSharedMemorySize, 160 * 1024 - 1024);
    if (e == hipSuccess) e = hipFuncSetAttribute((const void *)k_sparse_frame<false, PhaseClock>, hipFuncAttributeMaxDynamicSharedMemorySize, 160 * 1024 - 1024);
    return e;
}

template <int FMT>
__global__ void __launch_bounds__(256) k_luma8(const uint8_t *src, size_t pitch, size_t frame_stride, uint8_t *dst, int W, int H,
                                               int n_frames)
{
    const size_t plane = (size_t)W * (size_t)H, n = plane * (size_t)n_frames;
    for (size_t i = (size_t)blockIdx.x * blockDim.x + threadIdx.x; i < n; i += (size_t)gridDim.x * blockDim.x) {
        const size_t f = i / plane, r = i - f * plane;
        const size_t y = r / (size_t)W, x = r - y * (size_t)W;
        const uint8_t *row = src + f * frame_stride + y * pitch;
        uint32_t v;
        if (FMT == 1) {
            v = ((uint32_t)reinterpret_cast<const uint16_t *>(row)[x] + 128u) / 257u;
        } else {
            v = (2126u * row[3 * x] + 7152u * row[3 * x + 1] + 722u * row[3 * x + 2]) / 10000u;
        }
        dst[i] = (uint8_t)v;
    }
}

constexpr int FL_LA8 = 4, FL_RGBA8 = 5, FL_BGR8 = 6, FL_BGRA8 = 7, FL_RGB8P = 8, FL_LA16 = 9, FL_RGB16 = 10, FL_RGBA16 = 11;
constexpr int FL_ROWS = 4;

typedef uint32_t fl_u32x2 __attribute__((ext_vector_type(2), aligned(4)));
typedef uint32_t fl_u32x3 __attribute__((ext_vector_type(3), aligned(4)));
typedef uint32_t fl_u32x4 __attribute__((ext_vector_type(4), aligned(4)));

template <int LAYOUT>
struct FrontLayout {
    static constexpr bool in16 = LAYOUT >= FL_LA16;
    static constexpr int bpp = LAYOUT == FL_LA8 ? 2 : LAYOUT == FL_BGR8 ? 3 : LAYOUT == FL_RGB8P ? 1 : LAYOUT == FL_RGB16 ? 6
                             : LAYOUT == FL_RGBA16 ? 8 : 4;
    static constexpr int dwords = LAYOUT == FL_RGB8P ? 3 : bpp;
};

__device__ __forceinline__ uint32_t fl_weighted(uint32_t r, uint32_t g, uint32_t b) { return (2126u * r + 7152u * g + 722u * b) / 10000u; }

template <int LAYOUT>
__device__ __forceinline__ void fl_load4(const uint8_t *p, size_t plane, uint32_t (&d)[8])
{
    if (LAYOUT == FL_LA8) {
        const fl_u32x2 v = *reinterpret_cast<const fl_u32x2 *>(p);
        d[0] = v.x, d[1] = v.y;
    } else if (LAYOUT == FL_BGR8) {
        const fl_u32x3 v = *reinterpret_cast<const fl_u32x3 *>(p);
        d[0] = v.x, d[1] = v.y, d[2] = v.z;
    } else if (LAYOUT == FL_RGB8P) {
        d[0] = *reinterpret_cast<const uint32_t *>(p);
        d[1] = *reinterpret_cast<const uint32_t *>(p + plane);
        d[2] = *reinterpret_cast<const uint32_t *>(p + 2 * plane);
    } else {
        const fl_u32x4 v = *reinterpret_cast<const fl_u32x4 *>(p);
        d[0] = v.x, d[1] = v.y, d[2] = v.z, d[3] = v.w;
        if (LAYOUT == FL_RGB16) {
            const fl_u32x2 w = *reinterpret_cast<const fl_u32x2 *>(p + 16);
            d[4] = w.x, d[5] = w.y;
        } else if (LAYOUT == FL_RGBA16) {
            const fl_u32x4 w = *reinterpret_cast<const fl_u32x4 *>(p + 16);
            d[4] = w.x, d[5] = w.y, d[6] = w.z, d[7] = w.w;
        }
    }
}

template <int LAYOUT>
__device__ __forceinline__ uint32_t fl_luma_of(const uint32_t (&d)[8], int i)
{
    auto byte = [&](int k) { return (d[k >> 2] >> (8 * (k & 3))) & 0xffu; };
    auto half = [&](int k) { return (d[k >> 1] >> (16 * (k & 1))) & 0xffffu; };
    switch (LAYOUT) {
    case FL_LA8: return byte(2 * i);
    case FL_RGBA8: return fl_weighted(byte(4 * i), byte(4 * i + 1), byte(4 * i + 2));
    case FL_BGRA8: return fl_weighted(byte(4 * i + 2), byte(4 * i + 1), byte(4 * i));
    case FL_BGR8: return fl_weighted(byte(3 * i + 2), byte(3 * i + 1), byte(3 * i));
    case FL_RGB8P: return fl_weighted(byte(i), byte(4 + i), byte(8 + i));
    case FL_LA16: return half(2 * i);
    case FL_RGB16: return fl_weighted(half(3 * i), half(3 * i + 1), half(3 * i + 2));
    default: return fl_weighted(half(4 * i), half(4 * i + 1), half(4 * i + 2));
    }
}
// ... 377 lines not shown
    FrameCounters &ctr = a.ctr[frame];
    if (!frame_is_generic(a, ctr)) return;
    generic_frame(a, frame);
    if (threadIdx.x == 0) {
        __hip_atomic_store(&ctr.n_refined, 0u, __ATOMIC_RELAXED, __HIP_MEMORY_SCOPE_AGENT);
        __hip_atomic_store(&ctr.max_k_bits, 0u, __ATOMIC_RELAXED, __HIP_MEMORY_SCOPE_AGENT);
    }
    phase_barrier();
    const uint32_t n = min(__hip_atomic_load(&ctr.n_clusters, __ATOMIC_RELAXED, __HIP_MEMORY_SCOPE_AGENT), a.cap_roots);
    const size_t cbase = (size_t)frame * a.cap_roots;
    for (uint32_t i = threadIdx.x; i < n; i += blockDim.x) {
        float cx, cy;
        unsigned long long sx, sy;
        generic_sums(a, frame, i, sx, sy);
        cluster_centroid(&ctr.flags, a.clu_cnt[cbase + i], sx, sy, cx, cy);
        a.clu_sx[cbase + i] = __float_as_uint(cx);
        a.clu_sy[cbase + i] = __float_as_uint(cy);
    }
}

template <int HALF>
__global__ void __launch_bounds__(64) k_refine_clusters(ChainArgs a, const RefinePatchConsts *__restrict__ consts)
{
    __shared__ RefinePatchLds<HALF> s;
    const FrameSlot fs = frame_slot(a.n_frames, true);
    const int frame = fs.frame;
    FrameCounters &ctr = a.ctr[frame];
    const uint32_t g = threadIdx.x / REFINE_PATCH_LANES, l = threadIdx.x % REFINE_PATCH_LANES;
    uint32_t flags0 = ctr.flags, n0 = ctr.n_clusters;
    if (flags0 & (FLAG_CAND_OVERFLOW | FLAG_ROOT_OVERFLOW)) return;
    const uint32_t n = min(n0, a.cap_roots);
    const size_t cbase = (size_t)frame * a.cap_roots;
    const float *img = a.blur + (size_t)frame * (size_t)a.plane;
    const RefinePatchConsts *rc = consts + (HALF - 1);
    const RecSinkGlobal sink{&ctr.n_refined, &ctr.max_k_bits, &ctr.flags};
    for (uint32_t base = fs.slot * REFINE_PATCH_POINTS; base < n; base += fs.n_slots * REFINE_PATCH_POINTS) {
        const uint32_t i = base + g;
        const bool live = i < n;
        float rxf = 0.0f, ryf = 0.0f;
        bool inside = false;
        if (live) {
            rxf = roundf(__uint_as_float(a.clu_sx[cbase + i]));
            ryf = roundf(__uint_as_float(a.clu_sy[cbase + i]));
            inside = rxf >= (float)(2 * HALF) && ryf >= (float)(2 * HALF) && rxf <= 1073741824.0f && ryf <= 1073741824.0f;
            if (inside) inside = (int)ryf + 2 * HALF < a.H && (int)rxf + 2 * HALF < a.W;
        }
        const float *win = img;
        if (inside) win = img + (size_t)((int)ryf - 2 * HALF) * (size_t)a.W + ((int)rxf - 2 * HALF);
        refine_patch_body<HALF>(s, g, l, inside, win, (size_t)a.W, rc);
        if (inside && l == 0) {
            const float prm[6] = {s.prm[g][0], s.prm[g][1], s.prm[g][2], s.prm[g][3], s.prm[g][4], s.prm[g][5]};
            float rec[5];
            if (refine_tail(prm, rxf, ryf, rec) == POINT_REFINED) {
                const uint32_t o = atomicAdd(sink.n_refined, 1u);
                if (o < a.cap_roots) {
                    const uint32_t f6[6] = {a.clu_key[cbase + i],    __float_as_uint(rec[0]), __float_as_uint(rec[1]),
                                            __float_as_uint(rec[2]), __float_as_uint(rec[3]), __float_as_uint(rec[4])};
                    sink.put(a, frame, o, f6);
                    atomicMax(sink.max_k_bits, __float_as_uint(rec[2]));
                }
            }
        }
    }
}

int launch_generic_cluster(const ChainArgs &a, void *stream)
{
    hipLaunchKernelGGL(k_generic_cluster, dim3((unsigned)a.n_frames), dim3(1024), 0, (hipStream_t)stream, a);
    return hipGetLastError();
}

int launch_refine_clusters(const ChainArgs &a, const RefinePatchConsts *consts, int half, void *stream)
{
    if (!consts) return (int)hipErrorInvalidValue;
    const dim3 grid((unsigned)sparse_grid_x(a, 16, "AGX_G_REFINE") * (unsigned)a.n_frames), block(64);
    hipStream_t s = (hipStream_t)stream;
    switch (half) {
    case 1: hipLaunchKernelGGL((k_refine_clusters<1>), grid, block, 0, s, a, consts); break;
    case 2: hipLaunchKernelGGL((k_refine_clusters<2>), grid, block, 0, s, a, consts); break;
    case 3: hipLaunchKernelGGL((k_refine_clusters<3>), grid, block, 0, s, a, consts); break;
    case 4: hipLaunchKernelGGL((k_refine_clusters<4>), grid, block, 0, s, a, consts); break;
    default: return (int)hipErrorInvalidValue;
    }
    return hipGetLastError();
}

int launch_debug_resp(const ChainArgs &a, int frame, float *dst, void *stream)
{
    hipLaunchKernelGGL(k_debug_resp, dim3(1024), dim3(256), 0, (hipStream_t)stream,
                       a.blur + (size_t)frame * (size_t)a.plane, dst, a.W, a.H);
    return hipGetLastError();
}

template <int FMT>
__device__ __forceinline__ float luma32f_at(const uint8_t *__restrict__ rowp, int x)
{
    RawPx<FMT> r;
    if (FMT == 0) r.d[0] = rowp[x];
    else if (FMT == 1) r.d[0] = reinterpret_cast<const uint16_t *>(rowp)[x];
    else if (FMT == 2) r.d[0] = (uint32_t)rowp[3 * (size_t)x] | ((uint32_t)rowp[3 * (size_t)x + 1] << 8) | ((uint32_t)rowp[3 * (size_t)x + 2] << 16);
    else r.d[0] = reinterpret_cast<const uint32_t *>(rowp)[x];
#pragma unroll
    for (int i = 1; i < RawPx<FMT>::BPP; ++i) r.d[i] = 0u;
    float m[4];
    convert_px<FMT>(r, m);
    return m[0];
}

__device__ __forceinline__ void blur_taps4(const float *p, int stride, int taps, const float *__restrict__ w, float out[4])
{
    float v0 = p[0], v1 = p[stride], v2 = p[2 * stride];
    float a0 = 0.0f, a1 = 0.0f, a2 = 0.0f, a3 = 0.0f;
#pragma unroll 4
    for (int i = 0; i < taps; ++i) {
        const float v3 = p[(i + 3) * stride], wi = w[i];
        a0 += v0 * wi;
        a1 += v1 * wi;
        a2 += v2 * wi;
        a3 += v3 * wi;
        v0 = v1;
        v1 = v2;
        v2 = v3;
    }
    out[0] = a0;
    out[1] = a1;
    out[2] = a2;
    out[3] = a3;
}

template <int FMT>
__global__ void __launch_bounds__(256) k_gauss_blur(GaussBlurArgs a)
{
    extern __shared__ float gb_lds[];
    const int r = a.radius, taps = 2 * r + 1, W = a.W, H = a.H;
    const int rows_in = GB_TY + 2 * r, in_pitch = (GB_TX + 2 * r) | 1;
    float *tile = gb_lds, *hbuf = gb_lds + rows_in * in_pitch;
    const int t = (int)threadIdx.x, tx0 = (int)blockIdx.x * GB_TX;
    const uint8_t *frame = a.src + (size_t)blockIdx.z * (size_t)a.src_frame_stride;
    float *out = a.dst + (size_t)blockIdx.z * (size_t)a.dst_frame_stride;
    for (int ty0 = (int)blockIdx.y * GB_TY; ty0 < H; ty0 += (int)gridDim.y * GB_TY) {
        const int cols_in = GB_TX + 2 * r;
        for (int k = t; k < rows_in * cols_in; k += 256) {
            const int ry = k / cols_in, rx = k - ry * cols_in;
            const int y = min(max(ty0 - r + ry, 0), H - 1), x = min(max(tx0 - r + rx, 0), W - 1);
            tile[ry * in_pitch + rx] = luma32f_at<FMT>(frame + (size_t)y * (size_t)a.src_row_stride, x);
        }
        __syncthreads();
        for (int k = t; k < rows_in * (GB_TX / 4); k += 256) {
            const int cg = k / rows_in, ry = k - cg * rows_in;
            if (tx0 + 4 * cg >= W) continue;
            float o[4];
            blur_taps4(tile + ry * in_pitch + 4 * cg, 1, taps, a.w, o);
#pragma unroll
            for (int j = 0; j < 4; ++j) hbuf[ry * GB_HPITCH + 4 * cg + j] = o[j];
        }
        __syncthreads();
        for (int k = t; k < GB_TX * (GB_TY / 4); k += 256) {
            const int rg = k / GB_TX, cx = k - rg * GB_TX;
            const int x = tx0 + cx, y0 = ty0 + 4 * rg;
            if (x >= W || y0 >= H) continue;
            float o[4];
            blur_taps4(hbuf + 4 * rg * GB_HPITCH + cx, GB_HPITCH, taps, a.w, o);
#pragma unroll
            for (int j = 0; j < 4; ++j)
                if (y0 + j < H) out[(size_t)(y0 + j) * (size_t)a.dst_row_stride + (size_t)x] = o[j];
        }
// ... 295 lines not shown
```

### aprilgrid-rs_amd/csrc/detector.cpp

```cpp
#include <hip/hip_runtime_api.h>

#include <algorithm>
#include <cmath>
#include <cstdio>
#include <cstdlib>
#include <cstring>
#include <memory>
#include <new>
#include <string>
#include <system_error>
#include <vector>

#include "../../include/aprilgrid_amd.h"
#include "chain_kernels.h"
#include "decode_stages.h"
#include "detector_internal.h"
#include "host_tail.hpp"
#include "tail_kernels.h"

using namespace agx;

int agx::fail(agx_detector *d, int status, const std::string &msg)
{
    if (d) d->last_error = msg;
// ... 406 lines not shown
    return AGX_OK;
}

bool chain_any_sigma(const agx_detector *d)
{
    const float k1_sigma = 1.5f;
    return std::memcmp(&d->blur_sigma, &k1_sigma, sizeof k1_sigma) != 0;
}
int enqueue_any_sigma_front(agx_detector *d, const ChainArgs &a, hipStream_t st, bool with_response)
{
    GaussBlurArgs g{};
    g.src = a.frames;
    g.src_frame_stride = a.frame_stride;
    g.src_row_stride = a.row_stride;
    g.W = a.W;
    g.H = a.H;
    g.dst = a.blur;
    g.dst_row_stride = a.W;
    g.dst_frame_stride = a.plane;
    g.radius = d->front_radius;
    std::memcpy(g.w, d->front_w, sizeof(g.w));
    hipError_t e = (hipError_t)launch_gauss_blur(g, a.fmt, a.n_frames, st);
    if (e != hipSuccess) return fail(d, AGX_ERR_HIP, std::string("launch k_gauss_blur: ") + hipGetErrorString(e));
    if (!with_response) return AGX_OK;
    const EventPair ev = extra_timer_begin(d, st, XT_RESPONSE_FRONT);
    e = (hipError_t)launch_response_front(a, st);
    extra_timer_end(d, st, ev);
    if (e != hipSuccess) return fail(d, AGX_ERR_HIP, std::string("launch k_response_front: ") + hipGetErrorString(e));
    return AGX_OK;
}

int enqueue_chunk(agx_detector *d, int f0, int nf, hipStream_t st)
{
    ChainArgs a = d->args;
    const size_t F0 = (size_t)f0;
    a.n_frames = nf;
    a.frames += F0 * (size_t)a.frame_stride;
    a.blur += F0 * (size_t)a.plane;
    a.slot_plane += F0 * (size_t)a.plane;
    if (a.resp_dbg) a.resp_dbg += F0 * (size_t)a.plane;
    a.cand_max += F0 * (size_t)(a.mask_plane / 4);
    a.mask += F0 * (size_t)a.mask_plane;
    a.ctr += F0;
    if (a.ctr_next) a.ctr_next += F0;
    a.seeds += F0 * a.cap_roots;
    a.clu_key += F0 * a.cap_roots;
    a.clu_cnt += F0 * a.cap_roots;
    a.clu_sx += F0 * a.cap_roots;
    a.clu_sy += F0 * a.cap_roots;
    a.cand += F0 * a.cap_cand;
    a.parent += F0 * a.cap_cand;
    a.sumx += F0 * a.cap_cand;
    a.sumy += F0 * a.cap_cand;
    a.cnt += F0 * a.cap_cand;
    a.minidx += F0 * a.cap_cand;
    a.roots += F0 * a.cap_roots;
    a.refined += F0 * a.cap_roots;
    if (a.frame_table) a.frame_table += F0 * 4;
    int path = d->sparse_path;
    {
        const int forced = tuning_env("AGX_SPARSE_PATH", -1);
        if (forced >= 0 && forced <= 3) path = forced;
    }
    const int sparse_dbg = 32 | 64 | 128 | 256 | 2048 | 4096 | 8192 | 16384;
    const int cus = d->n_cus > 0 ? d->n_cus : 256, nearly = cus - cus / 4;
    if (path == 0) path = (nf >= nearly && (nf % cus == 0 || nf % cus >= nearly)) ? 3 : 1;
    const bool deferred = d->half_size_patch != 2 || d->chain_refine_general;
    const int chain_half = d->half_size_patch;
    const RefinePatchConsts *patch_consts = nullptr;
    if (deferred) {
        if (const int rc = ensure_patch_consts(d, &patch_consts)) return rc;
    }
    d->last_chain_refine = deferred ? 1 : 0;
    const bool fused = (path == 2 || path == 3) && !(a.dbg & sparse_dbg) && !deferred;
    d->last_sparse_frame = fused;
    d->last_sparse_path = fused ? path : 1;
    a.sparse_after_verify = fused && path == 3;
    const int plan_fused[] = {K_BLUR_HESSIAN, K_SPARSE}, plan_multi[] = {K_BLUR_HESSIAN, K_THRESHOLD, K_FLOOD_REFINE, K_RARE},
              plan_v_fe[] = {K_BLUR_HESSIAN, K_THRESHOLD, K_SPARSE};
    const int *plan = fused ? (path == 3 ? plan_v_fe : plan_fused) : plan_multi;
    const int n_plan = fused ? (path == 3 ? 3 : 2) : 4;
    const bool any_sigma = chain_any_sigma(d);
    d->last_chain_front = any_sigma ? 1 : 0;
    if (any_sigma) {
        const int rc = enqueue_any_sigma_front(d, a, st, true);
        if (rc) return rc;
    }
    for (int pi = any_sigma ? 1 : 0; pi < n_plan; ++pi) {
        const int k = plan[pi];
        EventPair ev{nullptr, nullptr, k};
        const bool timed = d->profiling >= 2 || (d->profiling == 1 && k == d->prof_kernel && d->prof_batches % (uint64_t)d->prof_stride == (uint64_t)d->prof_stride - 1);
        if (deferred && k == K_RARE) {
            hipError_t e = (hipError_t)launch_generic_cluster(a, st);
            if (e != hipSuccess) return fail(d, AGX_ERR_HIP, std::string("launch k_generic_cluster: ") + hipGetErrorString(e));
            e = (hipError_t)launch_refine_clusters(a, patch_consts, chain_half, st);
            if (e != hipSuccess) return fail(d, AGX_ERR_HIP, std::string("launch k_refine_clusters: ") + hipGetErrorString(e));
        }
        if (timed) {
            ev.a = get_event(d);
            ev.b = get_event(d);
            HIP_TRY(d, hipEventRecord(ev.a, st));
        }
        hipError_t e = (hipError_t)launch_kernel(k, a, d->rc, st, deferred);
        if (e != hipSuccess)
            return fail(d, AGX_ERR_HIP, std::string("launch ") + kKernelNames[k] + ": " + hipGetErrorString(e));
        if (timed) {
            HIP_TRY(d, hipEventRecord(ev.b, st));
            d->pending_events.push_back(ev);
        }
    }
    if (d->profiling) ++d->prof_batches;
    return AGX_OK;
}

int enqueue_chain(agx_detector *d)
{
    ChainArgs &a = d->args;
    const int p = d->ctr_cur ^ 1;
    const size_t need = (size_t)a.n_frames + 1;
    hipStreamCaptureStatus cap = hipStreamCaptureStatusNone;
    (void)hipStreamIsCapturing(d->stream, &cap);
    const bool capturing = cap == hipStreamCaptureStatusActive;
    if (capturing) {
        HIP_TRY(d, (hipError_t)launch_clear_counters(d->d_ctr[p], need, d->stream));
    } else if (d->ctr_cleared[p] < need) {
        HIP_TRY(d, hipMemsetAsync(d->d_ctr[p], 0, need * sizeof(FrameCounters), d->stream));
    }
    d->ctr_cleared[p] = 0;
    a.ctr = d->d_ctr[p];
    a.ctr_next = d->d_ctr[p ^ 1];
    a.total_out = &a.ctr[a.n_frames].min_key_inv;
    d->ctr_cleared[p ^ 1] = 0;
    const int rc = enqueue_chunk(d, 0, a.n_frames, d->stream);
    if (rc) return rc;
    d->ctr_cleared[p ^ 1] = capturing ? 0 : need;
    d->ctr_cur = p;
    d->batch = BATCH_SADDLES;
    return AGX_OK;
}

int enqueue_blur_only(agx_detector *d)
{
    ChainArgs &a = d->args;
    const int p = d->ctr_cur ^ 1;
    const size_t need = (size_t)a.n_frames + 1;
    hipStreamCaptureStatus cap = hipStreamCaptureStatusNone;
    (void)hipStreamIsCapturing(d->stream, &cap);
    if (cap == hipStreamCaptureStatusActive) {
        HIP_TRY(d, (hipError_t)launch_clear_counters(d->d_ctr[p], need, d->stream));
    } else if (d->ctr_cleared[p] < need) {
        HIP_TRY(d, hipMemsetAsync(d->d_ctr[p], 0, need * sizeof(FrameCounters), d->stream));
    }
    d->ctr_cleared[0] = d->ctr_cleared[1] = 0;
    a.ctr = d->d_ctr[p];
    a.ctr_next = d->d_ctr[p ^ 1];
    a.total_out = &a.ctr[a.n_frames].min_key_inv;
    if (chain_any_sigma(d)) {
        const int rc = enqueue_any_sigma_front(d, a, d->stream, false);
        if (rc) return rc;
        d->ctr_cur = p;
        return AGX_OK;
    }
    hipError_t e = (hipError_t)launch_kernel(K_BLUR_HESSIAN, a, d->rc, d->stream);
    if (e != hipSuccess) return fail(d, AGX_ERR_HIP, std::string("launch ") + kKernelNames[K_BLUR_HESSIAN] + ": " + hipGetErrorString(e));
    d->ctr_cur = p;
    return AGX_OK;
// ... 190 lines not shown
{
    return agx_guard(det, [&]() -> int {
    if (!det) return AGX_ERR_ARG;
    if (edge_bits) *edge_bits = det->fam.edge;
    if (border_bits) *border_bits = det->fam.border;
    if (hamming_distance) *hamming_distance = det->fam.hamming;
    if (codes) *codes = det->fam.codes;
    if (n_codes) *n_codes = det->fam.n_codes;
    return AGX_OK;
    });
}

int agx_detector_set_limits(agx_detector *det, uint32_t max_candidates, uint32_t max_clusters, uint32_t max_saddles)
{
    return agx_guard(det, [&]() -> int {
    if (!det) return AGX_ERR_ARG;
    if (max_candidates >= (1u << 30) || max_saddles > (1u << 24)) return AGX_ERR_ARG;
    det->lim_cand = max_candidates;
    det->lim_roots = max_clusters;
    det->lim_out = max_saddles;
    return AGX_OK;
    });
}

int agx_detector_set_blur_sigma(agx_detector *det, float sigma)
{
    return agx_guard(det, [&]() -> int {
    if (!det) return AGX_ERR_ARG;
    if (!blur_sigma_ok(sigma)) return fail(det, AGX_ERR_ARG, "sigma must be positive and finite with ceil(2 sigma) <= 16");
    det->blur_sigma = sigma;
    det->front_radius = make_blur_weights(sigma, det->front_w);
    return AGX_OK;
    });
}

int agx_detector_get_blur_sigma(const agx_detector *det, float *sigma)
{
    return agx_guard(det, [&]() -> int {
    if (!det || !sigma) return AGX_ERR_ARG;
    *sigma = det->blur_sigma;
    return AGX_OK;
    });
}

int agx_detector_set_half_size_patch(agx_detector *det, int half_size_patch)
{
    return agx_guard(det, [&]() -> int {
    if (!det) return AGX_ERR_ARG;
    if (half_size_patch < 1 || half_size_patch > REFINE_PATCH_MAX_HALF) return fail(det, AGX_ERR_ARG, "half_size_patch must be in 1 .. 4");
    det->half_size_patch = half_size_patch;
    return AGX_OK;
    });
}

int agx_detector_get_half_size_patch(const agx_detector *det, int *half_size_patch)
{
    return agx_guard(det, [&]() -> int {
    if (!det || !half_size_patch) return AGX_ERR_ARG;
    *half_size_patch = det->half_size_patch;
    return AGX_OK;
    });
}

int agx_detector_set_stream(agx_detector *det, void *hip_stream, int external)
{
    return agx_guard(det, [&]() -> int {
    if (!det) return AGX_ERR_ARG;
    HIP_TRY(det, hipSetDevice(det->device));
    HIP_TRY(det, hipStreamSynchronize(det->stream));
    harvest_events(det);
    det->stream = external ? (hipStream_t)hip_stream : det->own_stream;
    return AGX_OK;
    });
}

int agx_detector_set_option(agx_detector *det, const char *name, int value)
{
    return agx_guard(det, [&]() -> int {
    if (!det || !name) return AGX_ERR_ARG;
    if (!std::strcmp(name, "force_generic")) det->force_generic = value != 0;
    else if (!std::strcmp(name, "k1_rows_per_segment")) det->k1_rows = value > 0 ? value : 0;
    else if (!std::strcmp(name, "sparse_path")) det->sparse_path = value >= 0 && value <= 3 ? value : 0;
    else if (!std::strcmp(name, "debug_ablation")) det->dbg = value;
    else if (!std::strcmp(name, "store_response")) det->store_resp = value != 0;
    else if (!std::strcmp(name, "refine_general_kernel")) det->refine_general_kernel = value != 0;
    else if (!std::strcmp(name, "chain_refine_general")) det->chain_refine_general = value != 0;
    else if (!std::strcmp(name, "profile_stride")) det->prof_stride = value > 1 ? value : 1;
    else if (!std::strcmp(name, "profile_kernel")) det->prof_kernel = value >= 0 && value < K_COUNT ? value : K_BLUR_HESSIAN;
    else if (!std::strcmp(name, "device_tail")) {
        if (value > 0) {
            const uint64_t mismatches = libm_check_once();
            if (mismatches) {
                det->device_tail = 0;
                return fail(det, AGX_ERR_STATE, "device_tail: this C library's atan2f is not the routine the device tail restates (" +
                                                    std::to_string(mismatches) + " of 2^20 inputs differ); the host tail stays in use");
            }
        }
        det->device_tail = value > 0 ? 1 : (value < 0 ? -1 : 0);
    }
    else if (!std::strcmp(name, "tail_debug_band")) det->tail_debug_band_mdeg = value > 0 ? std::min(value, 30000) : 0;
    else if (!std::strcmp(name, "reload_tuning_env")) tuning_env_reload();
    else if (!std::strcmp(name, "tail_threads")) {
        const int n = value < 1 ? 1 : (value > 64 ? 64 : value);
        if (n != det->tail_threads) {
            if (det->tail_workers) destroy_tail_workers(det->tail_workers);
            det->tail_workers = nullptr;
            det->tail_threads = 1;
            det->tail_workers = create_tail_workers(n);
            det->tail_threads = n;
        }
    } else return fail(det, AGX_ERR_ARG, std::string("unknown option ") + name);
    return AGX_OK;
    });
}

int agx_detector_get_option(const agx_detector *det, const char *name, int *value)
{
    return agx_guard(det, [&]() -> int {
    if (!det || !name || !value) return AGX_ERR_ARG;
    const ChainArgs &a = det->args;
    if (!std::strcmp(name, "force_generic")) *value = det->force_generic;
    else if (!std::strcmp(name, "store_response")) *value = det->store_resp;
    else if (!std::strcmp(name, "debug_ablation")) *value = det->dbg;
    else if (!std::strcmp(name, "tail_threads")) *value = det->tail_threads;
    else if (!std::strcmp(name, "device_tail")) *value = det->device_tail;
    else if (!std::strcmp(name, "tail_debug_band")) *value = det->tail_debug_band_mdeg;
    else if (!std::strcmp(name, "last_find_boards_frames")) *value = det->last_find_frames;
    else if (!std::strcmp(name, "last_find_boards_handed_back")) *value = det->last_find_handed_back;
    else if (!std::strcmp(name, "last_grow_boards_frames")) *value = det->last_grow_frames;
    else if (!std::strcmp(name, "last_grow_boards_handed_back")) *value = det->last_grow_handed_back;
    else if (!std::strcmp(name, "last_init_quads_frames")) *value = det->last_init_frames;
    else if (!std::strcmp(name, "last_init_quads_handed_back")) *value = det->last_init_handed_back;
    else if (!std::strcmp(name, "last_device_tail_frames")) *value = det->last_tail_frames;
    else if (!std::strcmp(name, "last_device_tail_fallbacks")) *value = det->last_tail_fallbacks;
    else if (!std::strcmp(name, "last_device_tail_uncertain")) *value = det->last_tail_uncertain;
    else if (!std::strcmp(name, "k1_rows_per_segment")) *value = a.rows_per_seg;
    else if (!std::strcmp(name, "sparse_path")) *value = det->sparse_path;
    else if (!std::strcmp(name, "last_sparse_path")) *value = det->last_sparse_path;
    else if (!std::strcmp(name, "last_chain_front")) *value = det->last_chain_front;
    else if (!std::strcmp(name, "refine_general_kernel")) *value = det->refine_general_kernel;
    else if (!std::strcmp(name, "chain_refine_general")) *value = det->chain_refine_general;
    else if (!std::strcmp(name, "last_chain_refine")) *value = det->last_chain_refine;
    else if (!std::strcmp(name, "last_response_front_us")) *value = det->last_extra_us[XT_RESPONSE_FRONT];
    else if (!std::strcmp(name, "last_clusters_front_us")) *value = det->last_extra_us[XT_PLANE_FRONT];
    else if (!std::strcmp(name, "last_clusters_emit_us")) *value = det->last_extra_us[XT_EMIT_CLUSTERS];
    else if (!std::strcmp(name, "last_refine_kernel")) *value = det->last_refine_kernel;
    else if (!std::strcmp(name, "k1_segments")) *value = a.n_segs;
    else if (!std::strcmp(name, "k1_strips")) *value = a.n_strips;
    else if (!std::strcmp(name, "k1_strip_columns")) *value = a.strip_cols;
    else return AGX_ERR_ARG;
    return AGX_OK;
    });
}

int agx_detector_sync(agx_detector *det)
{
    return agx_guard(det, [&]() -> int {
    if (!det) return AGX_ERR_ARG;
    HIP_TRY(det, hipSetDevice(det->device));
    HIP_TRY(det, hipStreamSynchronize(det->stream));
    return AGX_OK;
    });
}

static int batch_enqueue_impl(agx_detector *det, const void *d_frames, int n_frames, int width, int height,
                              size_t row_stride_bytes, size_t frame_stride_bytes, int format, void *d_saddles,
                              uint32_t saddle_capacity, void *d_frame_table, bool blur_only = false)
{
    if (!det) return AGX_ERR_ARG;
    FrameBatch b{d_frames, n_frames, width, height, row_stride_bytes, frame_stride_bytes, format};
    int rc = check_frame_batch(det, b, { 2,  true,  true,  true,  true});
    if (rc) return rc;
    begin_batch(det);
    HIP_TRY(det, hipSetDevice(det->device));
    rc = ensure_workspace(det, n_frames, width, height);
    if (rc) return rc;
    if (format_front(format)) {
        if ((rc = front_luma_plane(det, b))) return rc;
        det->front_src = d_frames;
        det->front_format = format;
        det->front_frames = n_frames;
    }
    d_frames = b.frames;
    row_stride_bytes = b.row_stride;
    frame_stride_bytes = b.frame_stride;
    format = b.format;
    const bool byte_rows = ((row_stride_bytes | (uintptr_t)d_frames | (n_frames > 1 ? frame_stride_bytes : 0)) & 3) != 0;
    ChainArgs &a = det->args;
    a.frames = (const uint8_t *)d_frames;
    a.frame_stride = (long long)frame_stride_bytes;
    a.row_stride = (int)row_stride_bytes;
    a.byte_rows = byte_rows ? 1 : 0;
    a.fmt = format;
    a.W = width;
    a.H = height;
    a.n_frames = n_frames;
    a.plane = (long long)width * height;
    std::memcpy(a.w, det->blur_w, sizeof(a.w));
    a.min_angle = det->params.min_saddle_angle;
    a.max_angle = det->params.max_saddle_angle;
    if (d_saddles) {
        a.out = (float *)d_saddles;
        a.out_total_cap = saddle_capacity;
        a.frame_table = (uint32_t *)d_frame_table;
        det->external_out = true;
    } else {
        det->out_in_host = n_frames == 1 && det->h_out_dev != nullptr && det->h_table_dev != nullptr;
        a.out = det->out_in_host ? det->h_out_dev : det->d_out_internal;
        a.out_total_cap = (uint32_t)std::min<size_t>((size_t)n_frames * a.cap_out, 0xffffffffu);
        a.frame_table = det->out_in_host ? det->h_table_dev : nullptr;
        det->external_out = false;
    }
    a.force_generic = det->force_generic;
    a.dbg = det->dbg;
    a.wave_times = ((det->dbg & 4096) && (size_t)n_frames * (size_t)a.plane * 4 >= 3 * WAVE_TIMES_STRIDE * 16)
                       ? reinterpret_cast<unsigned long long *>(a.slot_plane) : nullptr;
    a.resp_dbg = nullptr;
    det->resp_stored = false;
    if (det->store_resp) {
        const size_t need = (size_t)n_frames * (size_t)a.plane * sizeof(float);
        a.resp_dbg = static_cast<float *>(side_ensure(det, SB_RESP_STORE, need, 0));
        if (!a.resp_dbg) return fail(det, AGX_ERR_HIP, "hipMalloc: response planes");
        HIP_TRY(det, hipMemsetAsync(a.resp_dbg, 0, need, det->stream));
        det->resp_stored = true;
    }
    if (!plan_k1(a, det->k1_rows)) return fail(det, AGX_ERR_ARG, "unsupported frame geometry");
    if (blur_only) return enqueue_blur_only(det);
    return enqueue_chain(det);
}

int agx_saddles_batch_enqueue(agx_detector *det, const void *d_frames, int n_frames, int width, int height,
                              size_t row_stride_bytes, size_t frame_stride_bytes, int format)
{
    return agx_guard(det, [&]() -> int {
    return batch_enqueue_impl(det, d_frames, n_frames, width, height, row_stride_bytes, frame_stride_bytes, format,
                              nullptr, 0, nullptr);
    });
}

int agx_saddles_batch_enqueue_to(agx_detector *det, const void *d_frames, int n_frames, int width, int height,
                                 size_t row_stride_bytes, size_t frame_stride_bytes, int format, void *d_saddles,
                                 uint32_t saddle_capacity, void *d_frame_table)
{
    return agx_guard(det, [&]() -> int {
    if (!d_saddles || !d_frame_table || ((uintptr_t)d_saddles & 3) || ((uintptr_t)d_frame_table & 3))
        return fail(det, AGX_ERR_ARG, "null or misaligned output buffers");
    return batch_enqueue_impl(det, d_frames, n_frames, width, height, row_stride_bytes, frame_stride_bytes, format,
                              d_saddles, saddle_capacity, d_frame_table);
    });
}

static int saddles_fetch_impl(agx_detector *det, agx_saddle *out, uint32_t cap_per_frame, uint32_t *counts, int *frame_status)
{
    return agx_guard(det, [&]() -> int {
    if (!det || !counts || (!out && cap_per_frame)) return fail(det, AGX_ERR_ARG, "null output");
    if (!chain_in_flight(det)) return fail(det, AGX_ERR_STATE, "no batch enqueued");
    if (det->external_out) return fail(det, AGX_ERR_STATE, "last batch wrote to caller-owned device buffers");
    HIP_TRY(det, hipSetDevice(det->device));
    const ChainArgs &a = det->args;
    const size_t F = (size_t)a.n_frames;
    bool have_counters = false;
    if (det->out_in_host) {
        HIP_TRY(det, hipStreamSynchronize(det->stream));
        have_counters = counters_of_row(det->h_table, det->h_ctr[0]);
        *det->h_total = det->h_table[0] + det->h_table[1];
    }
    bool out_fetched = det->out_in_host;
    if (!have_counters && !det->out_in_host && det->h_table_dev && det->h_out_dev && F + 1 <= det->h_table_rows) {
        hipError_t e = (hipError_t)launch_publish(a, (uint32_t)std::min<size_t>(det->h_out_records, 0xffffffffu), det->h_table_dev, det->h_out_dev, det->stream);
        if (e != hipSuccess) return fail(det, AGX_ERR_HIP, std::string("k_publish: ") + hipGetErrorString(e));
        HIP_TRY(det, hipStreamSynchronize(det->stream));
        bool bad = false;
        for (size_t f = 0; f < F; ++f)
            if (!counters_of_row(det->h_table + 4 * f, det->h_ctr[f])) bad = true;
        *det->h_total = det->h_table[4 * F];
        have_counters = !bad;
        out_fetched = true;
    }
    if (!have_counters) {
        HIP_TRY(det, hipMemcpyAsync(det->h_ctr, a.ctr, F * sizeof(FrameCounters), hipMemcpyDeviceToHost, det->stream));
        HIP_TRY(det, hipMemcpyAsync(det->h_total, a.total_out, sizeof(uint32_t), hipMemcpyDeviceToHost, det->stream));
        HIP_TRY(det, hipStreamSynchronize(det->stream));
    }
    harvest_events(det);
    const uint32_t total = *det->h_total;
    if (total > det->h_out_records) return fail(det, AGX_ERR_HIP, "compact output counter out of range");
    if (total && !out_fetched) {
        HIP_TRY(det, hipMemcpyAsync(det->h_out, a.out, (size_t)total * 5 * sizeof(float), hipMemcpyDeviceToHost,
                                    det->stream));
        HIP_TRY(det, hipStreamSynchronize(det->stream));
    }
    int first_bad = AGX_OK;
    for (size_t f = 0; f < F; ++f) {
        const FrameCounters &c = det->h_ctr[f];
        const int st = frame_status_of(c, cap_per_frame);
        counts[f] = c.n_out;
// ... 710 lines not shown
    if (cap < 2 * *radius + 1) return AGX_ERR_CAPACITY;
    make_blur_weights(sigma, weights);
    return AGX_OK;
    });
}

int agx_debug_refine_constants(int half_size_patch, float *cone, float *pmat, int cap_points, int *n_points)
{
    return agx_guard(nullptr, [&]() -> int {
    if (!cone || !pmat || !n_points || half_size_patch < 1 || half_size_patch > REFINE_PATCH_MAX_HALF) return AGX_ERR_ARG;
    const int ks = 2 * half_size_patch + 1;
    *n_points = ks * ks;
    if (cap_points < *n_points) return AGX_ERR_CAPACITY;
    RefinePatchConsts rc;
    make_refine_patch_consts(half_size_patch, rc);
    std::memcpy(cone, rc.cone, (size_t)*n_points * sizeof(float));
    std::memcpy(pmat, rc.pmat, (size_t)*n_points * 6 * sizeof(float));
    return AGX_OK;
    });
}

}

static int clusters_check_args(agx_detector *det, const float *plane, int n_frames, int width, int height, size_t row_stride_bytes,
                               size_t frame_stride_bytes, uint32_t clusters_per_frame, const agx_cluster_info *d_clusters,
                               const void *d_points, const uint32_t *d_counts, const uint32_t *d_status)
{
    const bool any = d_clusters || d_counts || d_status, all = d_clusters && d_counts && d_status;
    if (any != all) return fail(det, AGX_ERR_ARG, "d_clusters, d_counts and d_status: all or none");
    if (!clusters_per_frame || clusters_per_frame > EMIT_CLUSTERS_MAX) return fail(det, AGX_ERR_ARG, "clusters_per_frame must be in 1 .. 16384");
    if (((uintptr_t)d_clusters | (uintptr_t)d_points | (uintptr_t)d_counts | (uintptr_t)d_status) & 3)
        return fail(det, AGX_ERR_ARG, "the result buffers must be 4-byte aligned");
    return check_frame_batch(det, {plane, n_frames, width, height, row_stride_bytes, frame_stride_bytes, AGX_LF32},
                             { 2,  true,  true,  false,  false});
}

static int clusters_enqueue_impl(agx_detector *det, const float *d_response, int n_frames, int width, int height, size_t row_stride_bytes,
                                 size_t frame_stride_bytes, uint32_t clusters_per_frame, agx_cluster_info *d_clusters, void *d_points,
                                 uint32_t *d_counts, uint32_t *d_status)
{
    if (!det) return AGX_ERR_ARG;
    if (const int rc = clusters_check_args(det, d_response, n_frames, width, height, row_stride_bytes, frame_stride_bytes, clusters_per_frame,
                                           d_clusters, d_points, d_counts, d_status))
        return rc;
    const bool all = d_clusters != nullptr;
    const size_t slots = (size_t)n_frames * clusters_per_frame;
    HIP_TRY(det, hipSetDevice(det->device));
    begin_batch(det);
    if (const int rc = ensure_workspace(det, n_frames, width, height)) return rc;
    EmitClustersArgs e{};
    e.per_frame = clusters_per_frame;
    if (!all) {
        if (!side_ensure(det, SB_CLUSTERS_ROWS, slots * sizeof(agx_cluster_info), 0) || !side_ensure(det, SB_CLUSTERS_COUNTS, (size_t)n_frames * 4, 0) ||
            !side_ensure(det, SB_CLUSTERS_STATUS, (size_t)n_frames * 4, 0) || (!d_points && !side_ensure(det, SB_CLUSTERS_POINTS, slots * sizeof(agx_point), 0)))
            return fail(det, AGX_ERR_HIP, "hipMalloc: cluster rows");
        e.rows = det->side[SB_CLUSTERS_ROWS].ptr<uint32_t>();
        e.counts = det->side[SB_CLUSTERS_COUNTS].ptr<uint32_t>();
        e.status = det->side[SB_CLUSTERS_STATUS].ptr<uint32_t>();
        e.points = d_points ? static_cast<float *>(d_points) : det->side[SB_CLUSTERS_POINTS].ptr<float>();
    } else {
        e.rows = reinterpret_cast<uint32_t *>(d_clusters);
        e.counts = d_counts;
        e.status = d_status;
        e.points = static_cast<float *>(d_points);
    }
    ChainArgs &a = det->args;
    a.frames = reinterpret_cast<const uint8_t *>(d_response);
    a.frame_stride = (long long)frame_stride_bytes;
    a.row_stride = (int)row_stride_bytes;
    a.byte_rows = 0;
    a.fmt = AGX_LF32;
    a.W = width;
    a.H = height;
    a.n_frames = n_frames;
    a.plane = (long long)width * height;
    a.min_angle = det->params.min_saddle_angle;
    a.max_angle = det->params.max_saddle_angle;
    a.out = det->d_out_internal;
    a.out_total_cap = (uint32_t)std::min<size_t>((size_t)n_frames * a.cap_out, 0xffffffffu);
    a.frame_table = nullptr;
    det->external_out = false;
    det->out_in_host = false;
    a.force_generic = det->force_generic;
    a.sparse_after_verify = 0;
    a.dbg = 0;
    a.wave_times = nullptr;
    a.resp_dbg = nullptr;
    det->resp_stored = false;
    const int p = det->ctr_cur ^ 1;
    const size_t need = (size_t)n_frames + 1;
    hipStreamCaptureStatus cap = hipStreamCaptureStatusNone;
    (void)hipStreamIsCapturing(det->stream, &cap);
    if (cap == hipStreamCaptureStatusActive) {
        HIP_TRY(det, (hipError_t)launch_clear_counters(det->d_ctr[p], need, det->stream));
    } else if (det->ctr_cleared[p] < need) {
        HIP_TRY(det, hipMemsetAsync(det->d_ctr[p], 0, need * sizeof(FrameCounters), det->stream));
    }
    det->ctr_cleared[0] = det->ctr_cleared[1] = 0;
    a.ctr = det->d_ctr[p];
    a.ctr_next = det->d_ctr[p ^ 1];
    a.total_out = &a.ctr[n_frames].min_key_inv;
    det->ctr_cur = p;
    const PlaneFrontArgs front{d_response, (long long)(frame_stride_bytes / 4), (long long)(row_stride_bytes / 4)};
    const EventPair ev_front = extra_timer_begin(det, det->stream, XT_PLANE_FRONT);
    hipError_t err = (hipError_t)launch_plane_front(a, front, det->stream);
    extra_timer_end(det, det->stream, ev_front);
    if (err != hipSuccess) return fail(det, AGX_ERR_HIP, std::string("launch k_plane_front: ") + hipGetErrorString(err));
    err = (hipError_t)launch_kernel(K_THRESHOLD, a, det->rc, det->stream, true);
    if (err != hipSuccess) return fail(det, AGX_ERR_HIP, std::string("launch k_verify_seeds: ") + hipGetErrorString(err));
    err = (hipError_t)launch_kernel(K_FLOOD_REFINE, a, det->rc, det->stream, true);
    if (err != hipSuccess) return fail(det, AGX_ERR_HIP, std::string("launch k_flood_refine: ") + hipGetErrorString(err));
    err = (hipError_t)launch_generic_cluster(a, det->stream);
    if (err != hipSuccess) return fail(det, AGX_ERR_HIP, std::string("launch k_generic_cluster: ") + hipGetErrorString(err));
    const EventPair ev_emit = extra_timer_begin(det, det->stream, XT_EMIT_CLUSTERS);
    err = (hipError_t)launch_emit_clusters(a, e, det->stream);
    extra_timer_end(det, det->stream, ev_emit);
    if (err != hipSuccess) return fail(det, AGX_ERR_HIP, std::string("launch k_emit_clusters: ") + hipGetErrorString(err));
    det->batch = BATCH_CLUSTERS;
    det->clusters.results = all ? RESULTS_CALLER : RESULTS_HOST;
    det->clusters.n_frames = n_frames;
    det->clusters.clusters_per_frame = clusters_per_frame;
    det->clusters.d_points = all ? nullptr : reinterpret_cast<const agx_point *>(e.points);
    return AGX_OK;
}

static int clusters_fetch_impl(agx_detector *det, agx_cluster_info *clusters, void *points, uint32_t *counts, uint32_t *status)
{
    if (!det) return AGX_ERR_ARG;
    if (const int other = refuse_other_batch(det, BATCH_CLUSTERS)) return other;
    const ClustersPending b = det->clusters;
    const bool to_host = b.results == RESULTS_HOST;
    if (to_host && (!clusters || !counts || !status)) return fail(det, AGX_ERR_ARG, "null output");
    HIP_TRY(det, hipSetDevice(det->device));
    det->batch = BATCH_NONE;
    if (to_host) {
        const size_t F = (size_t)b.n_frames;
        HIP_TRY(det, hipMemcpyAsync(counts, det->side[SB_CLUSTERS_COUNTS].payload, F * 4, hipMemcpyDeviceToHost, det->stream));
        HIP_TRY(det, hipMemcpyAsync(status, det->side[SB_CLUSTERS_STATUS].payload, F * 4, hipMemcpyDeviceToHost, det->stream));
        HIP_TRY(det, hipStreamSynchronize(det->stream));
        const agx_cluster_info *d_rows = det->side[SB_CLUSTERS_ROWS].ptr<agx_cluster_info>();
        const agx_point *d_pts = points ? b.d_points : nullptr;
        for (size_t f = 0; f < F; ++f) {
            const size_t n = (status[f] & 0xffu) == AGX_CLUSTERS_OK ? std::min(counts[f], b.clusters_per_frame) : 0u, s0 = f * b.clusters_per_frame;
            if (!n) continue;
            HIP_TRY(det, hipMemcpyAsync(clusters + s0, d_rows + s0, n * sizeof(agx_cluster_info), hipMemcpyDeviceToHost, det->stream));
            if (d_pts) HIP_TRY(det, hipMemcpyAsync(static_cast<agx_point *>(points) + s0, d_pts + s0, n * sizeof(agx_point), hipMemcpyDeviceToHost, det->stream));
        }
    }
    HIP_TRY(det, hipStreamSynchronize(det->stream));
    harvest_events(det);
    return AGX_OK;
}

extern "C" {

int agx_clusters_enqueue(agx_detector *det, const float *d_response, int n_frames, int width, int height, size_t row_stride_bytes,
                         size_t frame_stride_bytes, uint32_t clusters_per_frame, agx_cluster_info *d_clusters, void *d_points,
                         uint32_t *d_counts, uint32_t *d_status)
{
    return agx_guard(det, [&]() -> int {
    return clusters_enqueue_impl(det, d_response, n_frames, width, height, row_stride_bytes, frame_stride_bytes, clusters_per_frame,
                                 d_clusters, d_points, d_counts, d_status);
    });
}

int agx_clusters_fetch(agx_detector *det, agx_cluster_info *clusters, void *points, uint32_t *counts, uint32_t *status)
// ... 360 lines not shown
    if (!det) return AGX_ERR_ARG;
    HIP_TRY(det, hipSetDevice(det->device));
    HIP_TRY(det, hipStreamSynchronize(det->stream));
    harvest_events(det);
    for (int k = 0; k < K_COUNT; ++k) {
        det->prof_ms[k] = 0.0;
        det->prof_launches[k] = 0;
    }
    det->prof_batches = 0;
    return AGX_OK;
    });
}

int agx_profile_read(agx_detector *det, const char **names, double *ms_total, uint64_t *launches)
{
    return agx_guard(det, [&]() -> int {
    if (!det) return AGX_ERR_ARG;
    HIP_TRY(det, hipSetDevice(det->device));
    HIP_TRY(det, hipStreamSynchronize(det->stream));
    harvest_events(det);
    for (int k = 0; k < AGX_N_KERNELS; ++k) {
        if (names) names[k] = k < K_COUNT ? kKernelNames[k] : nullptr;
        if (ms_total) ms_total[k] = k < K_COUNT ? det->prof_ms[k] : 0.0;
        if (launches) launches[k] = k < K_COUNT ? det->prof_launches[k] : 0;
    }
    return AGX_OK;
    });
}

int agx_detector_constants(const agx_detector *det, float *blur_w7, float *cone25, float *pmat150)
{
    return agx_guard(det, [&]() -> int {
    float w[7];
    RefineConsts rc;
    if (det) {
        std::memcpy(w, det->blur_w, sizeof w);
        rc = det->rc;
    } else {
        make_blur_weights(1.5f, w);
        make_refine_consts(rc);
    }
    if (blur_w7) std::memcpy(blur_w7, w, sizeof w);
    if (cone25) std::memcpy(cone25, rc.cone, sizeof rc.cone);
    if (pmat150) std::memcpy(pmat150, rc.pmat, sizeof rc.pmat);
    return AGX_OK;
    });
}

namespace {
int fetch_redzones(agx_detector *det, void *host_out, size_t cap_bytes, size_t *n_items)
{
    *n_items = 6;
    if (cap_bytes < 6 * sizeof(uint32_t)) return AGX_ERR_CAPACITY;
    HIP_TRY(det, hipSetDevice(det->device));
    HIP_TRY(det, hipStreamSynchronize(det->stream));
    const size_t rz = det->redzone;
    const uint64_t first_payload = det->device_allocs.empty() ? 0ull : (uint64_t)(uintptr_t)((char *)det->device_allocs[0] + rz);
    uint32_t v[6] = {0u, 0u, 0xffffffffu, 0u, (uint32_t)first_payload, (uint32_t)(first_payload >> 32)};
    std::vector<uint8_t> zone(rz);
    auto check = [&](const void *base, size_t bytes, bool host) -> int {
        const uint32_t index = v[0]++;
        for (int side = 0; rz && side < 2; ++side) {
            const char *src = (const char *)base + (side ? rz + bytes : 0);
            if (host) std::memcpy(zone.data(), src, rz);
            else HIP_TRY(det, hipMemcpy(zone.data(), src, rz, hipMemcpyDeviceToHost));
            for (size_t b = 0; b < rz; ++b)
                if (zone[b] != 0xA5 && v[1]++ == 0) {
                    v[2] = index;
                    v[3] = (uint32_t)(int32_t)(side ? (long long)(bytes + b) : (long long)b - (long long)rz);
                }
        }
        return AGX_OK;
    };
    for (size_t i = 0; i < det->device_allocs.size(); ++i)
        if (int rc = check(det->device_allocs[i], det->alloc_bytes[i], false)) return rc;
    for (const SideBuf &b : det->side)
        if (b.base)
            if (int rc = check(b.base, b.bytes, b.host)) return rc;
    std::memcpy(host_out, v, sizeof v);
    return AGX_OK;
}
}

int agx_debug_fetch(agx_detector *det, int frame, int what, void *host_out, size_t cap_bytes, size_t *n_items)
{
    return agx_guard(det, [&]() -> int {
    if (!det || !host_out || !n_items) return fail(det, AGX_ERR_ARG, "null argument");
    if (what == AGX_DBG_REDZONES) return fetch_redzones(det, host_out, cap_bytes, n_items);
    if (what == AGX_DBG_TAIL_TABLE_ADDR) {
        *n_items = 2;
        if (cap_bytes < 2 * sizeof(uint64_t)) return AGX_ERR_CAPACITY;
        const SideBuf &table = det->side[SB_TAIL_TABLE];
        if (!table.base) return fail(det, AGX_ERR_STATE, "no device tail has run on this handle");
        const uint64_t v[2] = {(uint64_t)(uintptr_t)table.payload, (uint64_t)table.bytes};
        std::memcpy(host_out, v, sizeof v);
        return AGX_OK;
    }
    if (!chain_in_flight(det)) return fail(det, AGX_ERR_STATE, "no batch enqueued");
    const ChainArgs &a = det->args;
    if (frame < 0 || frame >= a.n_frames) return fail(det, AGX_ERR_ARG, "frame out of range");
    HIP_TRY(det, hipSetDevice(det->device));
    HIP_TRY(det, hipStreamSynchronize(det->stream));
    const size_t plane = (size_t)a.plane;
    FrameCounters c;
    HIP_TRY(det, hipMemcpy(&c, a.ctr + frame, sizeof c, hipMemcpyDeviceToHost));
    switch (what) {
    case AGX_DBG_BLUR: {
        *n_items = plane;
        if (cap_bytes < plane * sizeof(float)) return AGX_ERR_CAPACITY;
        HIP_TRY(det, hipMemcpy(host_out, a.blur + (size_t)frame * plane, plane * sizeof(float), hipMemcpyDeviceToHost));
        return AGX_OK;
    }
    case AGX_DBG_RESP: {
        *n_items = plane;
        if (cap_bytes < plane * sizeof(float)) return AGX_ERR_CAPACITY;
        if (!det->resp_stored)
            return fail(det, AGX_ERR_STATE, "AGX_DBG_RESP needs option store_response=1 before the batch is enqueued");
        HIP_TRY(det, hipMemcpy(host_out, det->side[SB_RESP_STORE].ptr<float>() + (size_t)frame * plane, plane * sizeof(float), hipMemcpyDeviceToHost));
        return AGX_OK;
    }
    case AGX_DBG_RESP_RECOMPUTED: {
        *n_items = plane;
        if (cap_bytes < plane * sizeof(float)) return AGX_ERR_CAPACITY;
        float *d_resp = static_cast<float *>(side_ensure(det, SB_DBG_RESP, plane * sizeof(float), 0));
        if (!d_resp) return fail(det, AGX_ERR_HIP, "hipMalloc: response plane");
        hipError_t e = (hipError_t)launch_debug_resp(a, frame, d_resp, det->stream);
        if (e != hipSuccess) return fail(det, AGX_ERR_HIP, std::string("k_debug_resp: ") + hipGetErrorString(e));
        HIP_TRY(det, hipStreamSynchronize(det->stream));
        HIP_TRY(det, hipMemcpy(host_out, d_resp, plane * sizeof(float), hipMemcpyDeviceToHost));
        return AGX_OK;
    }
    case AGX_DBG_COUNTERS: {
        *n_items = 8;
        if (cap_bytes < 8 * sizeof(uint32_t)) return AGX_ERR_CAPACITY;
        const uint32_t v[8] = {c.flags, c.n_seeds, c.n_big, c.n_clusters + c.n_clusters2, c.n_cand, c.n_roots, c.n_refined, c.n_out};
        std::memcpy(host_out, v, sizeof v);
        return AGX_OK;
    }
    case 9: {
        const size_t lb = (size_t)a.W * (size_t)a.H;
        *n_items = lb;
        if (det->side[SB_LUMA_H].bytes < lb) return fail(det, AGX_ERR_STATE, "no device luma: agx_detect on an L16 / RGB8 image first");
        if (cap_bytes < lb) return AGX_ERR_CAPACITY;
        std::memcpy(host_out, det->side[SB_LUMA_H].payload, lb);
        return AGX_OK;
    }
    case 10: {
        if (!a.wave_times || frame < 1 || frame > 3) return fail(det, AGX_ERR_STATE, "wave timeline needs debug_ablation & 4096 on the last batch");
        const size_t n = std::min<size_t>(cap_bytes / 16, WAVE_TIMES_STRIDE);
        *n_items = n;
        HIP_TRY(det, hipMemcpy(host_out, a.wave_times + 2 * (size_t)(frame - 1) * WAVE_TIMES_STRIDE, n * 16, hipMemcpyDeviceToHost));
        return AGX_OK;
    }
    case 7: {
        *n_items = 20;
        if (cap_bytes < 20 * sizeof(uint32_t)) return AGX_ERR_CAPACITY;
        std::memcpy(host_out, c.stats, sizeof c.stats);
        return AGX_OK;
    }
    case AGX_DBG_MIN: {
        *n_items = 1;
        if (cap_bytes < sizeof(float)) return AGX_ERR_CAPACITY;
        uint32_t key = ~c.min_key_inv;
        uint32_t u = (key & 0x80000000u) ? (key & 0x7fffffffu) : ~key;
        std::memcpy(host_out, &u, sizeof u);
        return AGX_OK;
    }
    case AGX_DBG_CENTERS: {
        const uint32_t n = std::min(c.n_clusters + c.n_clusters2, a.cap_roots);
        *n_items = n;
        if (cap_bytes < (size_t)n * sizeof(agx_cluster_info)) return AGX_ERR_CAPACITY;
        std::vector<uint32_t> key(n), cnt(n), sx(n), sy(n);
        const size_t cb = (size_t)frame * a.cap_roots;
        HIP_TRY(det, hipMemcpy(key.data(), a.clu_key + cb, (size_t)n * 4, hipMemcpyDeviceToHost));
        HIP_TRY(det, hipMemcpy(cnt.data(), a.clu_cnt + cb, (size_t)n * 4, hipMemcpyDeviceToHost));
        HIP_TRY(det, hipMemcpy(sx.data(), a.clu_sx + cb, (size_t)n * 4, hipMemcpyDeviceToHost));
        HIP_TRY(det, hipMemcpy(sy.data(), a.clu_sy + cb, (size_t)n * 4, hipMemcpyDeviceToHost));
        std::vector<agx_cluster_info> info(n);
        for (uint32_t i = 0; i < n; ++i) {
            info[i].first_index = key[i];
            info[i].size = cnt[i];
            std::memcpy(&info[i].cx, &sx[i], 4);
            std::memcpy(&info[i].cy, &sy[i], 4);
        }
        std::sort(info.begin(), info.end(),
                  [](const agx_cluster_info &p, const agx_cluster_info &q) { return p.first_index < q.first_index; });
        std::memcpy(host_out, info.data(), (size_t)n * sizeof(agx_cluster_info));
        return AGX_OK;
    }
    case AGX_DBG_REFINED: {
        const uint32_t n = c.n_refined;
        *n_items = n;
        if (cap_bytes < (size_t)n * sizeof(agx_saddle)) return AGX_ERR_CAPACITY;
        std::vector<RefinedRec> rec(n);
        HIP_TRY(det, hipMemcpy(rec.data(), a.refined + (size_t)frame * a.cap_roots, (size_t)n * sizeof(RefinedRec),
                               hipMemcpyDeviceToHost));
        std::sort(rec.begin(), rec.end(), [](const RefinedRec &p, const RefinedRec &q) { return p.key < q.key; });
        agx_saddle *o = (agx_saddle *)host_out;
        for (uint32_t i = 0; i < n; ++i) o[i] = {rec[i].x, rec[i].y, rec[i].k, rec[i].theta, rec[i].phi};
        return AGX_OK;
    }
    default: return fail(det, AGX_ERR_ARG, "unknown debug item");
    }
    });
}

}
```

### aprilgrid-rs_amd/csrc/detector_internal.h

```cpp
#pragma once
#include <hip/hip_runtime_api.h>

#include <string>
#include <vector>

#include "../../include/aprilgrid_amd.h"
#include "chain_kernels.h"
#include "host_tail.hpp"

#define AGX_UPLOAD_STREAMS 3
#define HIP_TRY(det, expr)                                                                          \
    do {                                                                                            \
        hipError_t e_ = (expr);                                                                     \
        if (e_ != hipSuccess)                                                                       \
            return agx::fail((det), AGX_ERR_HIP, std::string(#expr) + ": " + hipGetErrorString(e_)); \
    } while (0)

namespace agx {
inline int format_px_bytes(int f)
{
    switch (f) {
    case AGX_L8: case AGX_RGB8P: return 1;
    case AGX_L16: case AGX_LA8: return 2;
    case AGX_RGB8: case AGX_BGR8: return 3;
// ... 95 lines not shown
    int min_side;
    bool lf32;
    bool lone_frame_stride;
    bool align16;
    bool front_rows;
};

struct EventPair {
    hipEvent_t a, b;
    int kernel;
};
enum { XT_RESPONSE_FRONT, XT_PLANE_FRONT, XT_EMIT_CLUSTERS, XT_COUNT };

struct SideBuf {
    void *base = nullptr;
    void *payload = nullptr;
    void *mapped = nullptr;
    size_t bytes = 0;
    bool host = false;
    template <class T> T *ptr() const { return static_cast<T *>(payload); }
    template <class T> T *dev() const { return static_cast<T *>(mapped); }
};
enum {
    SB_STAGE,
    SB_LUMA_D,
    SB_LUMA_H,
    SB_CODES,
    SB_TAGS,
    SB_TAIL_TABLE,
    SB_DTAGS,
    SB_DTABLE,
    SB_FETCH_LUMA,
    SB_FRONT,
    SB_RESP_STORE,
    SB_DBG_RESP,
    SB_REFINE_OUT,
    SB_REFINE_STATUS,
    SB_REFINE_POINTS,
    SB_REFINE_CONSTS,
    SB_DECODE_TAGS,
    SB_DECODE_STATUS,
    SB_DECODE_BITS,
    SB_DECODE_QUADS,
    SB_FIND_QUADS,
    SB_FIND_POINTS,
    SB_FIND_COUNTS,
    SB_FIND_STATUS,
    SB_FIND_SADDLES,
    SB_PLANES_BLUR,
    SB_PLANES_OUT,
    SB_CLUSTERS_ROWS,
    SB_CLUSTERS_POINTS,
    SB_CLUSTERS_COUNTS,
    SB_CLUSTERS_STATUS,
    SB_CLUSTERS_PLANE,
    SB_COUNT
};
}

struct agx_detector {
    int family = AGX_T36H11;
    agx::FamilyInfo fam{};
    agx_params params{};
    int device = 0;
    hipStream_t own_stream = nullptr;
    hipStream_t stream = nullptr;
    agx::RefineConsts rc{};
    float blur_w[7]{};
    float blur_sigma = 1.5f;
    int front_radius = 3;
    float front_w[2 * agx::GB_MAX_RADIUS + 1]{};
    int last_chain_front = 0;
    int half_size_patch = 2;
    int chain_refine_general = 0;
    int last_chain_refine = 0;
    uint32_t lim_cand = 0, lim_roots = 0, lim_out = 0;
    int force_generic = 0;
    int k1_rows = 0;
    int sparse_path = 0;
    bool last_sparse_frame = false;
    int last_sparse_path = 1;
    int n_cus = 0;
    int dbg = 0;
    int store_resp = 0;
    bool resp_stored = false;
    int ws_W = 0, ws_H = 0;

    agx::ChainArgs args{};
    size_t cap_frames = 0;
    long long cap_plane = 0;
    uint32_t alloc_cand = 0, alloc_roots = 0, alloc_out = 0;
    std::vector<void *> device_allocs;
    size_t redzone = 0;
    std::vector<size_t> alloc_bytes;
    agx::SideBuf side[agx::SB_COUNT];
    const void *front_src = nullptr;
    int front_format = -1, front_frames = 0;
    agx::FrameCounters *h_ctr = nullptr;
    size_t h_ctr_frames = 0;
    uint32_t *h_total = nullptr;
    float *h_out = nullptr;
    size_t h_out_records = 0;
    float *d_out_internal = nullptr;
    float *h_out_dev = nullptr;
    bool out_in_host = false;
    uint32_t *h_table = nullptr, *h_table_dev = nullptr;
    size_t h_table_rows = 0;
    size_t mask_words = 0;
    bool external_out = false;

    agx::FrameCounters *d_ctr[2] = {nullptr, nullptr};
    size_t ctr_cleared[2] = {0, 0};
    int ctr_cur = 0;

    int batch = agx::BATCH_NONE;
    int profiling = 0;
    int prof_stride = 1;
    int prof_kernel = agx::K_BLUR_HESSIAN;
    uint64_t prof_batches = 0;
    std::vector<agx::EventPair> pending_events;
    std::vector<hipEvent_t> free_events;
    double prof_ms[agx::K_COUNT]{};
    uint64_t prof_launches[agx::K_COUNT]{};

    hipStream_t upload_streams[AGX_UPLOAD_STREAMS] = {nullptr, nullptr, nullptr};
    bool upload_streams_ready = false;
    agx::TailWorkers *tail_workers = nullptr;
    int tail_threads = 1;
    agx::WorkerPool *pool = nullptr;
    int pool_threads = 0;
    std::vector<agx_saddle> scratch_saddles;

    int device_tail = -1;
    bool tail_ready = false;
    int tail_debug_band_mdeg = 0;
    size_t tail_frames = 0, dtail_frames = 0;
    uint32_t tail_tag_cap = 0, dtail_tag_cap = 0;
    int last_tail_frames = 0, last_tail_fallbacks = 0, last_tail_uncertain = 0;
    agx::DetectPending detect;
    agx::RefinePending refine;
    int refine_general_kernel = 0;
    int last_refine_kernel = 0;
    std::vector<agx::RefinePatchConsts> patch_consts;
    bool patch_consts_uploaded = false;
    std::vector<uint32_t> refine_host;
    agx::DecodePending decode;
    std::vector<uint64_t> decode_host;
    agx::FindPending find;
    int last_find_frames = 0, last_find_handed_back = 0;
    agx::ClustersPending clusters;
    agx::GrowPending grow;
    int last_grow_frames = 0, last_grow_handed_back = 0;
    agx::InitPending init;
    int last_init_frames = 0, last_init_handed_back = 0;
    int last_extra_us[agx::XT_COUNT]{};

    std::string last_error;
};

namespace agx {
int fail(agx_detector *d, int status, const std::string &msg);
inline void begin_batch(agx_detector *det)
{
    det->batch = BATCH_NONE;
    det->front_format = -1;
}
// ... 52 lines not shown
```

Baseline: 672,400 Mpix/s.

## Skip storing the blur plane and recompute blur from input bytes downstream

Adds a mode in which the first kernel no longer writes the f32 blurred plane. The verify and sparse-refine kernels instead recompute the separable 7-tap blur from the L8 input bytes, using a byte-to-weighted-float4 LUT. This removes a full f32 plane write and its later reads from HBM, at the cost of extra ALU work and more reads of the uint8 input. Debug fetches rebuild the plane on demand with a new debug blur kernel.

Result: no change. 671,800 Mpix/s, median of 2 (-0.1%).

```diff
diff --git a/aprilgrid-rs_amd/csrc/chain_kernels.h b/aprilgrid-rs_amd/csrc/chain_kernels.h
--- a/aprilgrid-rs_amd/csrc/chain_kernels.h
+++ b/aprilgrid-rs_amd/csrc/chain_kernels.h
@@ -99,6 +99,7 @@
     uint32_t out_total_cap;
     uint32_t *frame_table;
     float min_angle, max_angle;
+    int blur_in_plane;
 };
 
 int tuning_env(const char *name, int dflt);
@@ -142,6 +143,7 @@
 int init_device_kernels();
 
 int launch_debug_resp(const ChainArgs &a, int frame, float *dst, void *stream);
+int launch_debug_blur(const ChainArgs &a, int frame, void *stream);
 int launch_publish(const ChainArgs &a, uint32_t h_out_records, uint32_t *h_table_dev, float *h_out_dev, void *stream);
 int launch_clear_counters(FrameCounters *ctr, size_t n_records, void *stream);
 int launch_front_luma(const void *src, size_t row_stride, size_t frame_stride, int n_frames, int format, void *dst, int out8, int W,
diff --git a/aprilgrid-rs_amd/csrc/chain_kernels.hip b/aprilgrid-rs_amd/csrc/chain_kernels.hip
--- a/aprilgrid-rs_amd/csrc/chain_kernels.hip
+++ b/aprilgrid-rs_amd/csrc/chain_kernels.hip
@@ -748,6 +748,63 @@
     if (lane == 0 && !known_smaller) atomicMax(&ctr.min_key_inv, ~f32_order_key(run_min));
 }
 
+struct TapLut {
+    const float4 *t;
+    __device__ __forceinline__ float4 operator()(uint32_t v) const { return t[v]; }
+};
+struct TapMul {
+    const float *f;
+    float w0, w1, w2, w3;
+    __device__ __forceinline__ float4 operator()(uint32_t v) const
+    {
+        const float x = f[v];
+        return make_float4(x * w0, x * w1, x * w2, x * w3);
+    }
+};
+__device__ __forceinline__ void build_tap_lut(float4 *lut, const ChainArgs &a, uint32_t tid, uint32_t n_threads)
+{
+    for (uint32_t i = tid; i < 256u; i += n_threads) {
+        const float f = (float)i / 255.0f;
+        lut[i] = make_float4(f * a.w[0], f * a.w[1], f * a.w[2], f * a.w[3]);
+    }
+}
+template <int NX, typename TAPS, typename PX>
+__device__ __forceinline__ void reblur_hrow(const TAPS &taps, const PX &px, float (&h)[NX])
+{
+#pragma unroll
+    for (int i = 0; i < NX + 6; ++i) {
+        const float4 P = taps(px(i));
+#pragma unroll
+        for (int c = 0; c < NX; ++c) {
+            const int t = i - c;
+            if (t < 0 || t > 6) continue;
+            const int s = t <= 3 ? t : 6 - t;
+            const float e = s == 0 ? P.x : (s == 1 ? P.y : (s == 2 ? P.z : P.w));
+            h[c] = t == 0 ? e : h[c] + e;
+        }
+    }
+}
+template <int NX>
+__device__ __forceinline__ void reblur_push(float (&acc)[6][NX], const float (&h)[NX], const float (&w)[4], float (&out)[NX])
+{
+#pragma unroll
+    for (int c = 0; c < NX; ++c) {
+        const float p0 = h[c] * w[0], p1 = h[c] * w[1], p2 = h[c] * w[2], p3 = h[c] * w[3];
+        out[c] = acc[0][c] + p0;
+        acc[0][c] = acc[1][c] + p1;
+        acc[1][c] = acc[2][c] + p2;
+        acc[2][c] = acc[3][c] + p3;
+        acc[3][c] = acc[4][c] + p2;
+        acc[4][c] = acc[5][c] + p1;
+        acc[5][c] = p0;
+    }
+}
+__device__ __forceinline__ const uint8_t *reblur_row(const uint8_t *fbase, int row_stride, int H, int r)
+{
+    const int rr = r < 0 ? 0 : (r > H - 1 ? H - 1 : r);
+    return fbase + (size_t)rr * (size_t)row_stride;
+}
+
 __device__ __forceinline__ float det_at(const float *c, int W)
 {
     const float v11 = c[-W - 1], v12 = c[-W], v13 = c[-W + 1];
@@ -779,6 +836,52 @@
 #pragma unroll
         for (int q = 0; q < 4; ++q)
             if (!(d[q] < thr)) keep &= ~(1u << b[q]);
+    }
+    return keep;
+}
+
+template <typename TAPS>
+__device__ __forceinline__ uint32_t retest_bits_input(const ChainArgs &a, const uint8_t *fbase, const TAPS &taps, int x, int y0,
+                                                      uint32_t m0, float thr)
+{
+    const int W = a.W, H = a.H;
+    const float w[4] = {a.w[0], a.w[1], a.w[2], a.w[3]};
+    uint32_t keep = m0;
+    const int lo = m0 ? __ffs(m0) - 1 : 0;
+    const int n_rows = m0 ? (31 - __clz(m0)) - lo + 9 : 0;
+    int cx[9];
+#pragma unroll
+    for (int k = 0; k < 9; ++k) {
+        const int c = x - 4 + k;
+        cx[k] = c < 0 ? 0 : (c > W - 1 ? W - 1 : c);
+    }
+    float acc[6][3], up[3] = {0.0f, 0.0f, 0.0f}, mid[3] = {0.0f, 0.0f, 0.0f};
+#pragma unroll
+    for (int k = 0; k < 6; ++k)
+#pragma unroll
+        for (int c = 0; c < 3; ++c) acc[k][c] = 0.0f;
+    for (int i = 0; __any(i < n_rows); ++i) {
+        const uint8_t *rowp = reblur_row(fbase, a.row_stride, H, y0 + lo - 4 + i);
+        uint32_t b[9];
+#pragma unroll
+        for (int k = 0; k < 9; ++k) b[k] = rowp[cx[k]];
+        float h[3], dn[3];
+        reblur_hrow<3>(taps, [&](int k) { return b[k]; }, h);
+        reblur_push<3>(acc, h, w, dn);
+        if (i >= 8 && i < n_rows) {
+            const int bit = lo + i - 8;
+            const float t22 = mid[1] * 2.0f;
+            const float lxx = (mid[0] - t22) + mid[2];
+            const float lyy = (up[1] - t22) + dn[1];
+            const float lxy = (((up[2] - up[0]) + dn[0]) - dn[2]) * 0.25f;
+            const float d = lxx * lyy - lxy * lxy;
+            if (((m0 >> bit) & 1u) && !(d < thr)) keep &= ~(1u << bit);
+        }
+#pragma unroll
+        for (int c = 0; c < 3; ++c) {
+            up[c] = mid[c];
+            mid[c] = dn[c];
+        }
     }
     return keep;
 }
@@ -829,10 +932,12 @@
 }
 
 constexpr uint32_t K2_DBG_BITS = 32u | 64u | 128u | 256u | 2048u | 8192u;
-template <bool DBG, bool GRID3 = false>
+template <bool DBG, bool GRID3 = false, bool PLANE = true>
 __device__ __forceinline__ void verify_tiles(const ChainArgs &a, int frame, int first_tile, int tile_stride, uint32_t *s_keep,
                                              uint32_t *s_list)
 {
+    static_assert(VS_LIST >= 256, "the list's LDS holds the table of v / 255");
+    bool ftab_built = false;
     const uint32_t dbg = DBG ? a.dbg : 0u;
     FrameCounters &ctr = a.ctr[frame];
     uint32_t *mask = a.mask + (size_t)frame * (size_t)a.mask_plane;
@@ -921,7 +1026,28 @@
         for (int r = 0; r < VS_ROWS; ++r) keep[r] = m[r];
         uint32_t upbit = up_need ? 1u : 0u;
         const unsigned long long need_any = __ballot(needmask != 0u || up_retest);
-        if (need_any && !(dbg & 32)) {
+        if (!PLANE && need_any && !(dbg & 32)) {
+            float *ftab = reinterpret_cast<float *>(s_list);
+            if (!ftab_built) {
+                for (int i = lane; i < 256; i += 64) ftab[i] = (float)i / 255.0f;
+                wave_lds_sync();
+                ftab_built = true;
+            }
+            const TapMul taps{ftab, a.w[0], a.w[1], a.w[2], a.w[3]};
+            const uint8_t *fbase = a.frames + (size_t)frame * (size_t)a.frame_stride;
+            const uint32_t rows_any = wave_or_u32(needmask);
+#pragma unroll
+            for (int r = 0; r < VS_ROWS; ++r) {
+                if (!(rows_any & (1u << r))) continue;
+                const uint32_t mr = (needmask & (1u << r)) ? m[r] : 0u;
+                const uint32_t k = retest_bits_input(a, fbase, taps, x, (yb0 + r) * 32, mr, thr);
+                if (mr) keep[r] = k;
+            }
+            if (__any(up_retest)) {
+                const uint32_t k = retest_bits_input(a, fbase, taps, x, yb0 * 32 - 1, up_retest ? 1u : 0u, thr);
+                if (up_retest) upbit = k & 1u;
+            }
+        } else if (need_any && !(dbg & 32)) {
             const uint32_t rows_any = wave_or_u32(needmask);
             uint32_t n_list = 0;
             auto run_list = [&]() {
@@ -1028,7 +1154,7 @@
     }
 }
 
-template <bool DBG, bool GRID3 = false>
+template <bool DBG, bool GRID3 = false, bool PLANE = true>
 __global__ void __launch_bounds__(64 * VS_WAVES) AGX_VS_ATTR k_verify_seeds(ChainArgs a)
 {
     static_assert(!GRID3 || VS_WAVES == 1, "one tile per workgroup");
@@ -1037,13 +1163,13 @@
     const int wv = __builtin_amdgcn_readfirstlane((int)(threadIdx.x >> 6));
     const WaveTimer wt(a, K_THRESHOLD, DBG);
     if (GRID3) {
-        verify_tiles<DBG, true>(a, a.n_frames - 1 - (int)blockIdx.x, 0, 1, s_keep_all[0], s_list_all[0]);
+        verify_tiles<DBG, true, PLANE>(a, a.n_frames - 1 - (int)blockIdx.x, 0, 1, s_keep_all[0], s_list_all[0]);
         return;
     }
     FrameSlot fs = frame_slot(a.n_frames, true);
     fs.slot = fs.slot * VS_WAVES + (uint32_t)wv;
     fs.n_slots *= VS_WAVES;
-    verify_tiles<DBG>(a, fs.frame, (int)fs.slot, (int)fs.n_slots, s_keep_all[wv], s_list_all[wv]);
+    verify_tiles<DBG, false, PLANE>(a, fs.frame, (int)fs.slot, (int)fs.n_slots, s_keep_all[wv], s_list_all[wv]);
 }
 
 constexpr int VF_TB = 4;
@@ -1606,6 +1732,33 @@
     return lxx * lyy - lxy * lxy;
 }
 
+__global__ void __launch_bounds__(256) k_debug_blur(ChainArgs a, int frame)
+{
+    __shared__ float4 s_lut4[256];
+    build_tap_lut(s_lut4, a, threadIdx.x, blockDim.x);
+    __syncthreads();
+    const int W = a.W, H = a.H;
+    const uint8_t *fbase = a.frames + (size_t)frame * (size_t)a.frame_stride;
+    float *blur = a.blur + (size_t)frame * (size_t)a.plane;
+    const float w[4] = {a.w[0], a.w[1], a.w[2], a.w[3]};
+    const long long n = (long long)W * H;
+    for (long long i = (long long)blockIdx.x * blockDim.x + threadIdx.x; i < n; i += (long long)gridDim.x * blockDim.x) {
+        const int x = (int)(i % W), y = (int)(i / W);
+        float acc[6][1] = {{0.0f}, {0.0f}, {0.0f}, {0.0f}, {0.0f}, {0.0f}}, out[1] = {0.0f};
+#pragma unroll
+        for (int r = 0; r < 7; ++r) {
+            const uint8_t *rowp = reblur_row(fbase, a.row_stride, H, y - 3 + r);
+            float h[1];
+            reblur_hrow<1>(TapLut{s_lut4}, [&](int k) {
+                const int c = x - 3 + k;
+                return (uint32_t)rowp[c < 0 ? 0 : (c > W - 1 ? W - 1 : c)];
+            }, h);
+            reblur_push<1>(acc, h, w, out);
+        }
+        blur[i] = out[0];
+    }
+}
+
 __global__ void k_debug_resp(const float *__restrict__ blur, float *__restrict__ resp, int W, int H)
 {
     const long long n = (long long)W * H;
@@ -1645,10 +1798,14 @@
     }
 };
 
-template <bool VEC, typename CLK, typename SINK, typename SUM>
+struct ReblurSrc {
+    const uint8_t *fbase;
+    const float4 *lut;
+};
+template <bool VEC, bool PLANE = true, typename CLK, typename SINK, typename SUM>
 __device__ __forceinline__ void refine_values(const ChainArgs &a, const RefineConsts &rc, int frame, const float *img, int W, int H,
                                               uint32_t key, uint32_t cn, SUM sx, SUM sy, const SINK &sink, float &cx,
-                                              float &cy, CLK &clk)
+                                              float &cy, CLK &clk, const ReblurSrc src = ReblurSrc{nullptr, nullptr})
 {
     if (sx >= (1u << 24) || sy >= (1u << 24)) atomicOr(sink.flags, FLAG_CENTROID_INEXACT);
     const float fn = (float)cn;
@@ -1679,14 +1836,60 @@
             }
         asm volatile("" ::: "memory");
     };
-    fetch(0, 5);
+    const int ix0 = round_x - 7, ibase = ix0 & ~3;
+    const bool in_fast = ix0 >= 0 && ibase + 20 <= W;
+    const uint32_t in_al = in_fast ? (uint32_t)(ix0 & 3) : 0u;
+    uint32_t in_raw[5][5];
+    float in_acc[6][9];
+    const float in_w[4] = {a.w[0], a.w[1], a.w[2], a.w[3]};
+    auto fetch_in = [&](int first) {
+        typedef uint32_t u32x4a __attribute__((ext_vector_type(4), aligned(4)));
+#pragma unroll
+        for (int k = 0; k < 5; ++k) {
+            const uint8_t *rowp = reblur_row(src.fbase, a.row_stride, H, round_y - 7 + first + k);
+            if (in_fast) {
+                const u32x4a q = *reinterpret_cast<const u32x4a *>(rowp + ibase);
+                in_raw[k][0] = q[0];
+                in_raw[k][1] = q[1];
+                in_raw[k][2] = q[2];
+                in_raw[k][3] = q[3];
+                in_raw[k][4] = *reinterpret_cast<const uint32_t *>(rowp + ibase + 16);
+            } else {
+#pragma unroll
+                for (int q = 0; q < 5; ++q) in_raw[k][q] = 0u;
+#pragma unroll
+                for (int i = 0; i < 15; ++i) {
+                    const int c = ix0 + i;
+                    in_raw[k][i >> 2] |= (uint32_t)rowp[c < 0 ? 0 : (c > W - 1 ? W - 1 : c)] << (8 * (i & 3));
+                }
+            }
+        }
+        asm volatile("" ::: "memory");
+    };
+    auto push_in = [&](int ir, float (&out)[9]) __attribute__((always_inline)) {
+        const int k = ir % 5;
+        uint32_t d[4];
+#pragma unroll
+        for (int q = 0; q < 4; ++q) d[q] = __builtin_amdgcn_alignbyte(in_raw[k][q + 1], in_raw[k][q], in_al);
+        float h[9];
+        reblur_hrow<9>(TapLut{src.lut}, [&](int i) { return (d[i >> 2] >> (8 * (i & 3))) & 0xffu; }, h);
+        reblur_push<9>(in_acc, h, in_w, out);
+    };
+    if constexpr (PLANE) {
+        fetch(0, 5);
+    } else {
+#pragma unroll
+        for (int q = 0; q < 6; ++q)
+#pragma unroll
+            for (int c = 0; c < 9; ++c) in_acc[q][c] = 0.0f;
+    }
     if (CLK::on) {
         asm volatile("s_waitcnt vmcnt(0)" ::: "memory");
         clk.mark(11);
     }
 #pragma unroll
     for (int wr = 0; wr < 9; ++wr) {
-        if (wr == 5) {
+        if (PLANE && wr == 5) {
             clk.mark(12);
             fetch(5, 4);
             if (CLK::on) {
@@ -1696,7 +1899,13 @@
         }
         float v[9];
         const int k = wr < 5 ? wr : wr - 5;
-        if (VEC) {
+        if constexpr (!PLANE) {
+#pragma unroll
+            for (int ir = (wr == 0 ? 0 : wr + 6); ir <= wr + 6; ++ir) {
+                if (ir % 5 == 0) fetch_in(ir);
+                push_in(ir, v);
+            }
+        } else if (VEC) {
             const rowload_t q0 = raw[k][0], q1 = raw[k][1 % NQ], q2 = raw[k][2 % NQ];
             const bool s1 = (al & 1) != 0, s2 = (al & 2) != 0;
             const float u0 = s1 ? q0[1 % (VEC ? 4 : 1)] : q0[0], u1 = s1 ? q0[2 % (VEC ? 4 : 1)] : q0[1 % (VEC ? 4 : 1)], u2 = s1 ? q0[3 % (VEC ? 4 : 1)] : q0[2 % (VEC ? 4 : 1)], u3 = s1 ? q1[0] : q0[3 % (VEC ? 4 : 1)];
@@ -1784,17 +1993,17 @@
     cy = (float)sy / fn;
 }
 
-template <bool VEC>
+template <bool VEC, bool PLANE = true>
 __device__ __forceinline__ void refine_cluster(const ChainArgs &a, const RefineConsts &rc, int frame, size_t cbase,
                                                const float *img, int W, int H, uint32_t s, uint32_t *n_refined,
-                                               uint32_t *max_k_bits)
+                                               uint32_t *max_k_bits, const ReblurSrc src = ReblurSrc{nullptr, nullptr})
 {
     float cx, cy;
     NoClock clk;
     const RecSinkGlobal sink{n_refined, max_k_bits, &a.ctr[frame].flags};
     unsigned long long sx, sy;
     generic_sums(a, frame, s, sx, sy);
-    refine_values<VEC>(a, rc, frame, img, W, H, a.clu_key[cbase + s], a.clu_cnt[cbase + s], sx, sy, sink, cx, cy, clk);
+    refine_values<VEC, PLANE>(a, rc, frame, img, W, H, a.clu_key[cbase + s], a.clu_cnt[cbase + s], sx, sy, sink, cx, cy, clk, src);
     a.clu_sx[cbase + s] = __float_as_uint(cx);
     a.clu_sy[cbase + s] = __float_as_uint(cy);
 }
@@ -2082,9 +2291,9 @@
     return h;
 }
 
-template <bool EMIT_ONLY = false>
+template <bool EMIT_ONLY = false, bool PLANE = true>
 __device__ __forceinline__ void rare_frame(const ChainArgs &a, const RefineConsts &rc, int frame, uint32_t *lds_u, uint32_t lds_entries,
-                                           uint32_t *s_misc3, const FrameHead &head)
+                                           uint32_t *s_misc3, const FrameHead &head, const ReblurSrc src = ReblurSrc{nullptr, nullptr})
 {
     uint32_t &s_count = s_misc3[0], &s_offset = s_misc3[1], &s_fits = s_misc3[2];
     FrameCounters &ctr = a.ctr[frame];
@@ -2103,7 +2312,7 @@
         if (!(flags & (FLAG_CAND_OVERFLOW | FLAG_ROOT_OVERFLOW))) {
             const uint32_t n = min(__hip_atomic_load(&ctr.n_clusters, __ATOMIC_RELAXED, __HIP_MEMORY_SCOPE_AGENT), a.cap_roots);
             for (uint32_t i = threadIdx.x; i < n; i += blockDim.x)
-                refine_cluster<false>(a, rc, frame, cbase, img, a.W, a.H, i, &ctr.n_refined, &ctr.max_k_bits);
+                refine_cluster<false, PLANE>(a, rc, frame, cbase, img, a.W, a.H, i, &ctr.n_refined, &ctr.max_k_bits, src);
         }
         phase_barrier();
     }
@@ -2287,10 +2496,12 @@
 static_assert(SF_WORDS * 4 <= 160 * 1024 - 1024, "fits a CU's LDS");
 enum : int { SFM_SEEDS = 0, SFM_FLAGS = 1, SFM_CLUSTERS = 2, SFM_REFINED = 3, SFM_MAXK = 4, SFM_BIG = 5, SFM_EMIT = 8, SFM_RARE = 12 };
 
-template <bool VEC, typename CLK>
+template <bool VEC, typename CLK, bool PLANE = true>
 __global__ void __launch_bounds__(1024) k_sparse_frame(ChainArgs a, RefineConsts rc, uint32_t lds_entries)
 {
     extern __shared__ __attribute__((aligned(16))) uint32_t lds_u[];
+    __shared__ float4 s_lut4[PLANE ? 1 : 256];
+    if constexpr (!PLANE) build_tap_lut(s_lut4, a, threadIdx.x, 1024u);
     const int frame = a.n_frames - 1 - (int)blockIdx.x;
     const uint32_t t = threadIdx.x;
     const int lane = (int)(t & 63u);
@@ -2308,6 +2519,7 @@
     const size_t cbase = (size_t)frame * a.cap_roots;
     const float *img = a.blur + (size_t)frame * (size_t)a.plane;
     const RecSinkLds sink{&misc[SFM_REFINED], &misc[SFM_MAXK], &misc[SFM_FLAGS], lds_u + SF_REC};
+    const ReblurSrc src{a.frames + (size_t)frame * (size_t)a.frame_stride, s_lut4};
     if (a.sparse_after_verify) {
         if (t == 0) {
             misc[SFM_SEEDS] = __hip_atomic_load(&ctr.n_seeds, __ATOMIC_RELAXED, __HIP_MEMORY_SCOPE_AGENT);
@@ -2365,7 +2577,7 @@
             if (what == FLOOD_CLUSTER) {
                 const uint32_t o = atomicAdd(&misc[SFM_CLUSTERS], 1u);
                 float cx, cy;
-                refine_values<VEC>(a, rc, frame, img, a.W, a.H, p, cnt, sumx, sumy, sink, cx, cy, clk);
+                refine_values<VEC, PLANE>(a, rc, frame, img, a.W, a.H, p, cnt, sumx, sumy, sink, cx, cy, clk, src);
                 if (o < a.cap_roots) {
                     a.clu_key[cbase + o] = p;
                     a.clu_cnt[cbase + o] = cnt;
@@ -2394,7 +2606,7 @@
     if (generic || (!void_frame && n_ref > TAIL_CAP)) {
         if (t == 0) atomicOr(&ctr.flags, flags);
         phase_barrier();
-        rare_frame(a, rc, frame, lds_u + SF_MISC, lds_entries, &misc[SFM_RARE], load_frame_head(ctr));
+        rare_frame<false, PLANE>(a, rc, frame, lds_u + SF_MISC, lds_entries, &misc[SFM_RARE], load_frame_head(ctr), src);
         return;
     }
     emit_wide_lds(a, frame, void_frame ? 0u : n_ref, misc[SFM_MAXK], lds_u + SF_REC, lds_u + SF_R, &misc[SFM_EMIT], &misc[SFM_FLAGS], n_clu);
@@ -2478,6 +2690,12 @@
     const size_t k1_lds = (size_t)env_int("AGX_K1_LDS_KB", 0) * 1024;
     const bool small = a.plane * 4 < (1ll << 31) && (long long)a.H * a.row_stride < (1ll << 31);
     const bool a4 = (a.W & 3) == 0 && small && !a.byte_rows;
+    if (!a.blur_in_plane && !(a.dbg & 1)) {
+        ChainArgs k = a;
+        k.dbg |= 1;
+        k.blur_in_plane = 1;
+        return launch_k1<FMT>(k, st);
+    }
     const bool uf = !a4 && small && a.W >= 4 && env_int("AGX_K1_UNALIGNED_FAST", 1) != 0;
     if (uf) {
         if (a.resp_dbg) hipLaunchKernelGGL((k_blur_hessian<FMT, false, true, true>), grid, block, k1_lds, st, a);
@@ -2519,7 +2737,13 @@
         if (tiles > 512) tiles = 512;
         const int per_frame = (env_int("AGX_G_VERIFY", tiles) + VS_WAVES - 1) / VS_WAVES;
         dim3 grid((unsigned)per_frame * (unsigned)a.n_frames), block(64 * VS_WAVES);
-        if ((a.dbg & K2_DBG_BITS) || a.wave_times) hipLaunchKernelGGL(k_verify_seeds<true>, grid, block, 0, st, a);
+        const bool grid3 = VS_WAVES == 1 && env_int("AGX_G_VERIFY", 0) <= 0 && (n_yb + VS_ROWS - 1) / VS_ROWS <= 65535 && (a.W + VS_OWN - 1) / VS_OWN <= 65535;
+        if (!a.blur_in_plane) {
+            if (grid3)
+                hipLaunchKernelGGL((k_verify_seeds<false, VS_WAVES == 1, false>), dim3((unsigned)a.n_frames, (unsigned)((a.W + VS_OWN - 1) / VS_OWN), (unsigned)((n_yb + VS_ROWS - 1) / VS_ROWS)),
+                                   block, 0, st, a);
+            else hipLaunchKernelGGL((k_verify_seeds<false, false, false>), grid, block, 0, st, a);
+        } else if ((a.dbg & K2_DBG_BITS) || a.wave_times) hipLaunchKernelGGL(k_verify_seeds<true>, grid, block, 0, st, a);
         else if (VS_WAVES == 1 && env_int("AGX_G_VERIFY", 0) <= 0 && (n_yb + VS_ROWS - 1) / VS_ROWS <= 65535 && (a.W + VS_OWN - 1) / VS_OWN <= 65535)
             hipLaunchKernelGGL((k_verify_seeds<false, VS_WAVES == 1>), dim3((unsigned)a.n_frames, (unsigned)((a.W + VS_OWN - 1) / VS_OWN), (unsigned)((n_yb + VS_ROWS - 1) / VS_ROWS)),
                                block, 0, st, a);
@@ -2557,6 +2781,8 @@
         if (a.dbg & 262144) {
             if ((a.W & 3) == 0) hipLaunchKernelGGL((k_sparse_frame<true, PhaseClock>), grid, block, lds, st, a, rc, le);
             else hipLaunchKernelGGL((k_sparse_frame<false, PhaseClock>), grid, block, lds, st, a, rc, le);
+        } else if (!a.blur_in_plane) {
+            hipLaunchKernelGGL((k_sparse_frame<true, NoClock, false>), grid, block, lds, st, a, rc, le);
         } else if ((a.W & 3) == 0) hipLaunchKernelGGL((k_sparse_frame<true, NoClock>), grid, block, lds, st, a, rc, le);
         else hipLaunchKernelGGL((k_sparse_frame<false, NoClock>), grid, block, lds, st, a, rc, le);
         return hipGetLastError();
@@ -2572,6 +2798,7 @@
     if (e == hipSuccess) e = hipFuncSetAttribute((const void *)k_rare_emit_only, hipFuncAttributeMaxDynamicSharedMemorySize, 160 * 1024 - 1024);
     if (e == hipSuccess) e = hipFuncSetAttribute((const void *)k_sparse_frame<true, NoClock>, hipFuncAttributeMaxDynamicSharedMemorySize, 160 * 1024 - 1024);
     if (e == hipSuccess) e = hipFuncSetAttribute((const void *)k_sparse_frame<false, NoClock>, hipFuncAttributeMaxDynamicSharedMemorySize, 160 * 1024 - 1024);
+    if (e == hipSuccess) e = hipFuncSetAttribute((const void *)k_sparse_frame<true, NoClock, false>, hipFuncAttributeMaxDynamicSharedMemorySize, 160 * 1024 - 1024 - 4096);
     if (e == hipSuccess) e = hipFuncSetAttribute((const void *)k_sparse_frame<true, PhaseClock>, hipFuncAttributeMaxDynamicSharedMemorySize, 160 * 1024 - 1024);
     if (e == hipSuccess) e = hipFuncSetAttribute((const void *)k_sparse_frame<false, PhaseClock>, hipFuncAttributeMaxDynamicSharedMemorySize, 160 * 1024 - 1024);
     return e;
@@ -3115,6 +3342,14 @@
     case 4: hipLaunchKernelGGL((k_refine_clusters<4>), grid, block, 0, s, a, consts); break;
     default: return (int)hipErrorInvalidValue;
     }
+    return hipGetLastError();
+}
+
+int launch_debug_blur(const ChainArgs &a, int frame, void *stream)
+{
+    long long blocks = ((long long)a.W * a.H + 255) / 256;
+    if (blocks > 65535) blocks = 65535;
+    hipLaunchKernelGGL(k_debug_blur, dim3((unsigned)blocks), dim3(256), 0, (hipStream_t)stream, a, frame);
     return hipGetLastError();
 }
 
diff --git a/aprilgrid-rs_amd/csrc/detector.cpp b/aprilgrid-rs_amd/csrc/detector.cpp
--- a/aprilgrid-rs_amd/csrc/detector.cpp
+++ b/aprilgrid-rs_amd/csrc/detector.cpp
@@ -512,6 +512,12 @@
     const int n_plan = fused ? (path == 3 ? 3 : 2) : 4;
     const bool any_sigma = chain_any_sigma(d);
     d->last_chain_front = any_sigma ? 1 : 0;
+    const bool no_plane_legal = fused && path == 3 && a.fmt == AGX_L8 && (a.W & 3) == 0 && !a.byte_rows && a.plane * 4 < (1ll << 31) &&
+                                (long long)a.H * a.row_stride < (1ll << 31) && !any_sigma && !a.resp_dbg && a.dbg == 0 && !a.wave_times;
+    a.blur_in_plane = (d->blur_plane_store == 0 && no_plane_legal) ? 0 : 1;
+    d->last_blur_in_plane = a.blur_in_plane;
+    if (f0 == 0) d->batch_without_plane = false;
+    if (!a.blur_in_plane) d->batch_without_plane = true;
     if (any_sigma) {
         const int rc = enqueue_any_sigma_front(d, a, st, true);
         if (rc) return rc;
@@ -868,6 +874,7 @@
     else if (!std::strcmp(name, "k1_rows_per_segment")) det->k1_rows = value > 0 ? value : 0;
     else if (!std::strcmp(name, "sparse_path")) det->sparse_path = value >= 0 && value <= 3 ? value : 0;
     else if (!std::strcmp(name, "debug_ablation")) det->dbg = value;
+    else if (!std::strcmp(name, "blur_plane_store")) det->blur_plane_store = value == 0 ? 0 : (value == 1 ? 1 : -1);
     else if (!std::strcmp(name, "store_response")) det->store_resp = value != 0;
     else if (!std::strcmp(name, "refine_general_kernel")) det->refine_general_kernel = value != 0;
     else if (!std::strcmp(name, "chain_refine_general")) det->chain_refine_general = value != 0;
@@ -908,6 +915,8 @@
     if (!std::strcmp(name, "force_generic")) *value = det->force_generic;
     else if (!std::strcmp(name, "store_response")) *value = det->store_resp;
     else if (!std::strcmp(name, "debug_ablation")) *value = det->dbg;
+    else if (!std::strcmp(name, "blur_plane_store")) *value = det->blur_plane_store;
+    else if (!std::strcmp(name, "last_blur_in_plane")) *value = det->last_blur_in_plane;
     else if (!std::strcmp(name, "tail_threads")) *value = det->tail_threads;
     else if (!std::strcmp(name, "device_tail")) *value = det->device_tail;
     else if (!std::strcmp(name, "tail_debug_band")) *value = det->tail_debug_band_mdeg;
@@ -998,6 +1007,7 @@
         det->external_out = false;
     }
     a.force_generic = det->force_generic;
+    a.blur_in_plane = 1;
     a.dbg = det->dbg;
     a.wave_times = ((det->dbg & 4096) && (size_t)n_frames * (size_t)a.plane * 4 >= 3 * WAVE_TIMES_STRIDE * 16)
                        ? reinterpret_cast<unsigned long long *>(a.slot_plane) : nullptr;
@@ -1874,6 +1884,7 @@
     det->external_out = false;
     det->out_in_host = false;
     a.force_generic = det->force_generic;
+    a.blur_in_plane = 1;
     a.sparse_after_verify = 0;
     a.dbg = 0;
     a.wave_times = nullptr;
@@ -2400,6 +2411,15 @@
 }
 }
 
+static int fill_blur_plane(agx_detector *det, int frame)
+{
+    if (!det->batch_without_plane) return AGX_OK;
+    hipError_t e = (hipError_t)launch_debug_blur(det->args, frame, det->stream);
+    if (e != hipSuccess) return fail(det, AGX_ERR_HIP, std::string("k_debug_blur: ") + hipGetErrorString(e));
+    HIP_TRY(det, hipStreamSynchronize(det->stream));
+    return AGX_OK;
+}
+
 int agx_debug_fetch(agx_detector *det, int frame, int what, void *host_out, size_t cap_bytes, size_t *n_items)
 {
     return agx_guard(det, [&]() -> int {
@@ -2426,6 +2446,7 @@
     case AGX_DBG_BLUR: {
         *n_items = plane;
         if (cap_bytes < plane * sizeof(float)) return AGX_ERR_CAPACITY;
+        if (const int rc = fill_blur_plane(det, frame)) return rc;
         HIP_TRY(det, hipMemcpy(host_out, a.blur + (size_t)frame * plane, plane * sizeof(float), hipMemcpyDeviceToHost));
         return AGX_OK;
     }
@@ -2442,6 +2463,7 @@
         if (cap_bytes < plane * sizeof(float)) return AGX_ERR_CAPACITY;
         float *d_resp = static_cast<float *>(side_ensure(det, SB_DBG_RESP, plane * sizeof(float), 0));
         if (!d_resp) return fail(det, AGX_ERR_HIP, "hipMalloc: response plane");
+        if (const int rc = fill_blur_plane(det, frame)) return rc;
         hipError_t e = (hipError_t)launch_debug_resp(a, frame, d_resp, det->stream);
         if (e != hipSuccess) return fail(det, AGX_ERR_HIP, std::string("k_debug_resp: ") + hipGetErrorString(e));
         HIP_TRY(det, hipStreamSynchronize(det->stream));
diff --git a/aprilgrid-rs_amd/csrc/detector_internal.h b/aprilgrid-rs_amd/csrc/detector_internal.h
--- a/aprilgrid-rs_amd/csrc/detector_internal.h
+++ b/aprilgrid-rs_amd/csrc/detector_internal.h
@@ -201,6 +201,9 @@
     int last_sparse_path = 1;
     int n_cus = 0;
     int dbg = 0;
+    int blur_plane_store = -1;
+    int last_blur_in_plane = 1;
+    bool batch_without_plane = false;
     int store_resp = 0;
     bool resp_stored = false;
     int ws_W = 0, ws_H = 0;
```
